# XiSHEN0220/RANSAC-Flow

Measured on NVIDIA H100. Metric: image-pairs/sec at 480x640, nbIter=1k RANSAC, higher is better.
Workload: dtype f32-grade: fp16 hi/lo split operands and activations (22 significand bits), 3 wgmma MMAs per MAC, fp32 accumulate; fp16-split correlation; fp32/fp64 RANSAC

## Files before the change

### ransac-flow_b200/csrc/gemm_tc.cu

```cuda
#include <cuda.h>
#include <cuda_fp16.h>

#include <climits>
#include <mutex>
#include <unordered_map>

#include "common.cuh"
#include "tc_common.cuh"

namespace rf {

constexpr int K_TF32 = 0, K_F16 = 1, K_SPLIT = 2, K_TF32X3 = 3;
constexpr int MODE_CONV = 0, MODE_CORR = 1;
constexpr int O_F32 = 0, O_F16 = 1, O_SPLIT = 2;
constexpr int WG_THREADS = 288;

struct alignas(64) WgParams {
    CUtensorMap mapA[RF_MAX_IMGS];
    CUtensorMap mapA2[RF_MAX_IMGS];
    CUtensorMap mapY[RF_MAX_IMGS];
    CUtensorMap mapR[RF_MAX_IMGS];
    CUtensorMap mapB;
    CUtensorMap mapBlo;
    int nimg;
    int ntiles;
    int tile_start[RF_MAX_IMGS + 1];
    int tiles_x[RF_MAX_IMGS];
    int tw[RF_MAX_IMGS];
    int Ho[RF_MAX_IMGS], Wo[RF_MAX_IMGS];
    long long out_pix[RF_MAX_IMGS + 1];
    int R, S, pad, stride, Cin, Cout, relu, round_out;
    int dil;
    int kc1, stride2;
    long long plane;
    const float* bias;
    const void* residual;
    void* y;
    unsigned long long* rowbest;
    unsigned long long* colbest;
    int NA, NB;
};
static_assert(sizeof(WgParams) <= 32764, "kernel parameter space (CUDA 12.1+ large kernel parameters)");

template <int KIND, int BN, int MODE>
struct WgCfg {
    static constexpr int NPL = (KIND == K_SPLIT || KIND == K_TF32X3) ? 2 : 1;
    static constexpr int A_BYTES = NPL * TC_A_BYTES;
    static constexpr int B_PLANE = BN * 128;
    static constexpr int STAGE_BYTES = A_BYTES + NPL * B_PLANE;
    static constexpr bool ONE_CTA = MODE == MODE_CORR || NPL * BN >= 256;
    static constexpr int BUDGET = ONE_CTA ? 200 * 1024 : 100 * 1024;
    static constexpr int STAGES = BUDGET / STAGE_BYTES > 6 ? 6 : BUDGET / STAGE_BYTES;
    static constexpr int CTAS_PER_SM = ONE_CTA ? 1 : 2;
    static constexpr int SMEM_BYTES = STAGES * STAGE_BYTES + 1024  + 256 ;
    static_assert(STAGES >= 2 && SMEM_BYTES <= 227 * 1024, "shared memory");
};

__device__ __forceinline__ __half2 pack_sat(float a, float b) {
    uint32_t r;
    asm("cvt.rn.satfinite.f16x2.f32 %0, %1, %2;" : "=r"(r) : "f"(b), "f"(a));
    return *reinterpret_cast<__half2*>(&r);
}
__device__ __forceinline__ void split2(float a, float b, __half2& hi, __half2& lo) {
    hi = pack_sat(a, b);
    const float2 f = __half22float2(hi);
    lo = pack_sat((a - f.x) * 2048.f, (b - f.y) * 2048.f);
}

template <int KIND, int BN, int NACC>
__device__ __forceinline__ void mma_block(float (&acc)[NACC][BN / 2], uint32_t sa, uint32_t sb) {
    constexpr bool TF32 = KIND == K_TF32 || KIND == K_TF32X3;
#pragma unroll
    for (int k = 0; k < 4; ++k) {
        const uint64_t ah = wg_desc(sa + 32 * k), bh = wg_desc(sb + 32 * k);
        if constexpr (KIND == K_SPLIT || KIND == K_TF32X3) {
            const uint64_t al = wg_desc(sa + TC_A_BYTES + 32 * k), bl = wg_desc(sb + BN * 128 + 32 * k);
            float (&x)[BN / 2] = acc[NACC - 1];
            wgmma<TF32, BN>(x, al, bh);
            wgmma<TF32, BN>(x, ah, bl);
            wgmma<TF32, BN>(acc[0], ah, bh);
        } else {
            wgmma<TF32, BN>(acc[0], ah, bh);
        }
    }
}

template <int KIND, int BN, int MODE, int OUT>
__global__ void __launch_bounds__(WG_THREADS, WgCfg<KIND, BN, MODE>::CTAS_PER_SM)
wg_kernel(const __grid_constant__ WgParams p) {
    using Cfg = WgCfg<KIND, BN, MODE>;
    constexpr int STAGES = Cfg::STAGES;
    constexpr int BK = (KIND == K_TF32 || KIND == K_TF32X3) ? TC_BK : TC_BK_F16;
    constexpr int NACC = KIND == K_SPLIT ? 2 : 1;
    constexpr bool SLOT = MODE == MODE_CONV && OUT != O_F32;
    constexpr int BOX_BYTES = (OUT == O_SPLIT ? 2 : 1) * 128 * 128;
    static_assert(!SLOT || (BN / 64) * BOX_BYTES <= Cfg::STAGE_BYTES, "the output tile fits one stage");
    extern __shared__ uint8_t smem_raw[];
    uint8_t* smem = smem_raw + ((1024u - (smem_u32(smem_raw) & 1023u)) & 1023u);
    uint64_t* full = reinterpret_cast<uint64_t*>(smem + STAGES * Cfg::STAGE_BYTES);
    uint64_t* empty = full + STAGES;
    const int warp = threadIdx.x >> 5, lane = threadIdx.x & 31;
    const int kc = p.Cin / BK;
    const int KI = p.R * p.S * kc;

    const int t_first = MODE == MODE_CORR ? 0 : (int)blockIdx.x;
    const int t_step = MODE == MODE_CORR ? 1 : (int)gridDim.x;
    const int t_end = MODE == MODE_CORR ? 1 : p.ntiles;
    const int nt = (p.Cout + BN - 1) / BN;
    struct Tile { int img, tw, ox0, oy0, n0; };
    auto decode = [&](int t) {
        const int mtile = MODE == MODE_CORR ? (int)blockIdx.y : t / nt;
        const int ntile = MODE == MODE_CORR ? (int)blockIdx.x : t - mtile * nt;
        Tile T;
        T.img = 0;
#pragma unroll
        for (int j = 1; j < RF_MAX_IMGS; ++j) T.img += (j < p.nimg && mtile >= p.tile_start[j]) ? 1 : 0;
        const int tloc = mtile - p.tile_start[T.img];
        T.tw = p.tw[T.img];
        const int tyi = tloc / p.tiles_x[T.img], txi = tloc - tyi * p.tiles_x[T.img];
        T.ox0 = txi * T.tw;
        T.oy0 = tyi * (128 / T.tw);
        T.n0 = ntile * BN;
        return T;
    };
    auto boxes = [&](const Tile& T) { return BN == 64 || T.n0 + 64 >= p.Cout ? 1 : 2; };

    if (threadIdx.x == 0) {
        for (int s = 0; s < STAGES; ++s) { mbar_init(&full[s], 1); mbar_init(&empty[s], 256); }
        fence_barrier_init();
    }
    __syncthreads();

    if (warp == 8) {
        if (lane == 0) {
            tma_prefetch_desc(&p.mapB);
            uint32_t prefetched = 0;
            int st = 0;
            uint32_t ph = 0;
            for (int t = t_first; t < t_end; t += t_step) {
                const Tile T = decode(t);
                if (!((prefetched >> T.img) & 1u)) {
                    prefetched |= 1u << T.img;
                    tma_prefetch_desc(&p.mapA[T.img]);
                    if constexpr (SLOT) {
                        tma_prefetch_desc(&p.mapY[T.img]);
                        if (p.residual) tma_prefetch_desc(&p.mapR[T.img]);
                    }
                }
                for (int it = 0; it < KI; ++it) {
                    mbar_wait(&empty[st], ph ^ 1);
                    uint8_t* sa = smem + st * Cfg::STAGE_BYTES;
                    uint8_t* sb = sa + Cfg::A_BYTES;
                    mbar_expect_tx(&full[st], Cfg::STAGE_BYTES);
                    if constexpr (MODE == MODE_CORR) {
                        const int c0 = it * BK;
                        tma_load_3d(sa, &p.mapA[0], &full[st], c0, T.ox0, 0);
                        tma_load_3d(sa + TC_A_BYTES, &p.mapA2[0], &full[st], c0, T.ox0, 0);
                        tma_load_2d(sb, &p.mapB, &full[st], c0, T.n0);
                        tma_load_2d(sb + Cfg::B_PLANE, &p.mapBlo, &full[st], c0, T.n0);
                    } else {
                        const int tap = it / kc, cc = it - tap * kc;
                        const int r = tap / p.S, s = tap - r * p.S;
                        const int c0 = cc * BK, x = T.ox0 * p.stride + s * p.dil - p.pad, y = T.oy0 * p.stride + r * p.dil - p.pad;
                        const int kcol = tap * p.Cin + c0;
                        if constexpr (KIND == K_SPLIT) {
                            if (cc < p.kc1) tma_load_4d(sa, &p.mapA[T.img], &full[st], c0, x, y, 0);
                            else tma_load_4d(sa, &p.mapA2[T.img], &full[st], (cc - p.kc1) * BK, T.ox0 * p.stride2, T.oy0 * p.stride2, 0);
                            tma_load_3d(sb, &p.mapB, &full[st], kcol, T.n0, 0);
                        } else {
                            tma_load_3d(sa, &p.mapA[T.img], &full[st], c0, x, y);
                            tma_load_2d(sb, &p.mapB, &full[st], kcol, T.n0);
                        }
                    }
                    if (++st == STAGES) { st = 0; ph ^= 1; }
                }
                if constexpr (SLOT) {
                    mbar_wait(&empty[st], ph ^ 1);
                    if (p.residual) {
                        const int nb = boxes(T);
                        uint8_t* slot = smem + st * Cfg::STAGE_BYTES;
                        mbar_expect_tx(&full[st], nb * BOX_BYTES);
                        for (int b = 0; b < nb; ++b) {
                            if constexpr (OUT == O_SPLIT) tma_load_4d(slot + b * BOX_BYTES, &p.mapR[T.img], &full[st], T.n0 + 64 * b, T.ox0, T.oy0, 0);
                            else tma_load_3d(slot + b * BOX_BYTES, &p.mapR[T.img], &full[st], T.n0 + 64 * b, T.ox0, T.oy0);
                        }
                    } else {
                        mbar_arrive(&full[st]);
                    }
                    if (++st == STAGES) { st = 0; ph ^= 1; }
                }
            }
        }
        return;
    }

    const int g = warp >> 2;
    const int rbase = 64 * g + 16 * (warp & 3) + (lane >> 2);
    const int cbase = 2 * (lane & 3);
    auto before = [](int s) { return s == 0 ? STAGES - 1 : s - 1; };
    int st = 0;
    uint32_t ph = 0;
    bool stored = false;
    for (int t = t_first; t < t_end; t += t_step) {
        const Tile T = decode(t);
        float acc[NACC][BN / 2];
#pragma unroll
        for (int a = 0; a < NACC; ++a)
#pragma unroll
            for (int i = 0; i < BN / 2; ++i) acc[a][i] = 0.f;
        for (int it = 0; it < KI; ++it) {
            mbar_wait(&full[st], ph);
            const uint32_t sa = smem_u32(smem + st * Cfg::STAGE_BYTES);
            wg_fence();
            mma_block<KIND, BN, NACC>(acc, sa + g * (64 * 128), sa + Cfg::A_BYTES);
            wg_commit();
            wg_wait<1>();
            if (it > 0) {
                mbar_arrive(&empty[before(st)]);
            } else if (SLOT && stored) {
                if (threadIdx.x == 0) bulk_wait_read();
                mbar_arrive(&empty[before(st)]);
            }
            if (++st == STAGES) { st = 0; ph ^= 1; }
        }
        wg_wait<0>();
#pragma unroll
        for (int a = 0; a < NACC; ++a) wg_fence_regs(acc[a]);
        mbar_arrive(&empty[before(st)]);

        auto value = [&](int i) -> float {
            if constexpr (KIND == K_SPLIT) return fmaf(acc[1][i], 0.00048828125f, acc[0][i]);
            else return acc[0][i];
        };

        if constexpr (SLOT) {
            mbar_wait(&full[st], ph);
            uint8_t* slot = smem + st * Cfg::STAGE_BYTES;
#pragma unroll
            for (int h = 0; h < 2; ++h) {
                const int m = rbase + 8 * h;
#pragma unroll
                for (int j = 0; j < BN / 8; ++j) {
                    const int c = 8 * j + cbase, n = T.n0 + c;
                    if (n >= p.Cout) continue;
                    float v0 = value(4 * j + 2 * h), v1 = value(4 * j + 2 * h + 1);
                    if (p.bias) { v0 += __ldg(p.bias + n); v1 += __ldg(p.bias + n + 1); }
                    uint8_t* e = slot + (c >> 6) * BOX_BYTES + m * 128 + ((((c & 63) >> 3) ^ (m & 7)) << 4) + (c & 7) * 2;
                    if (p.residual) {
                        if constexpr (OUT == O_F16) {
                            const float2 r = __half22float2(*reinterpret_cast<const __half2*>(e));
                            v0 += r.x; v1 += r.y;
                        } else {
                            const float2 rh = __half22float2(*reinterpret_cast<const __half2*>(e));
                            const float2 rl = __half22float2(*reinterpret_cast<const __half2*>(e + 128 * 128));
                            v0 += fmaf(rl.x, 0.00048828125f, rh.x); v1 += fmaf(rl.y, 0.00048828125f, rh.y);
                        }
                    }
                    if (p.relu) { v0 = fmaxf(v0, 0.f); v1 = fmaxf(v1, 0.f); }
                    if constexpr (OUT == O_F16) {
                        *reinterpret_cast<__half2*>(e) = pack_sat(v0, v1);
                    } else {
                        __half2 hi, lo;
                        split2(v0, v1, hi, lo);
                        *reinterpret_cast<__half2*>(e) = hi;
                        *reinterpret_cast<__half2*>(e + 128 * 128) = lo;
                    }
                }
            }
            fence_proxy_async();
            asm volatile("bar.sync 1, 256;" ::: "memory");
            if (threadIdx.x == 0) {
                const int nb = boxes(T);
                for (int b = 0; b < nb; ++b) {
                    if constexpr (OUT == O_SPLIT) tma_store_4d(&p.mapY[T.img], slot + b * BOX_BYTES, T.n0 + 64 * b, T.ox0, T.oy0, 0);
                    else tma_store_3d(&p.mapY[T.img], slot + b * BOX_BYTES, T.n0 + 64 * b, T.ox0, T.oy0);
                }
                bulk_commit();
            }
            stored = true;
            if (++st == STAGES) { st = 0; ph ^= 1; }
        } else if constexpr (MODE == MODE_CONV) {
            const int img = T.img, tw = T.tw;
#pragma unroll
            for (int h = 0; h < 2; ++h) {
                const int m = rbase + 8 * h;
                const int py = m / tw, px = m - py * tw;
                const int oy = T.oy0 + py, ox = T.ox0 + px;
                if (oy >= p.Ho[img] || ox >= p.Wo[img]) continue;
                const long long pix = p.out_pix[img] + (long long)oy * p.Wo[img] + ox;
#pragma unroll
                for (int j = 0; j < BN / 8; ++j) {
                    const int n = T.n0 + 8 * j + cbase;
                    if (n >= p.Cout) continue;
                    const bool two = n + 1 < p.Cout;
                    float v0 = value(4 * j + 2 * h), v1 = value(4 * j + 2 * h + 1);
                    if (p.bias) { v0 += __ldg(p.bias + n); if (two) v1 += __ldg(p.bias + n + 1); }
                    const long long o = pix * p.Cout + n;
                    if (p.residual) {
                        const float* r = static_cast<const float*>(p.residual) + o;
                        v0 += __ldg(r); if (two) v1 += __ldg(r + 1);
                    }
                    if (p.relu) { v0 = fmaxf(v0, 0.f); v1 = fmaxf(v1, 0.f); }
                    if (p.round_out) { v0 = round_tf32(v0); v1 = round_tf32(v1); }
                    float* y = static_cast<float*>(p.y) + o;
                    if (two && (p.Cout & 1) == 0) *reinterpret_cast<float2*>(y) = make_float2(v0, v1);
                    else { y[0] = v0; if (two) y[1] = v1; }
                }
            }
        } else {
            const int n0 = T.n0;
            unsigned long long* sCol = reinterpret_cast<unsigned long long*>(smem);
            const int row0 = T.ox0 + rbase, row1 = row0 + 8;
            const bool rv0 = row0 < p.NA, rv1 = row1 < p.NA;
            unsigned long long rb0 = 0ull, rb1 = 0ull;
            asm volatile("bar.sync 1, 256;" ::: "memory");
#pragma unroll
            for (int j = 0; j < BN / 8; ++j) {
#pragma unroll
                for (int e = 0; e < 2; ++e) {
                    const int c = 8 * j + cbase + e, col = n0 + c;
                    const bool cv = col < p.NB;
                    const float s0 = value(4 * j + e), s1 = value(4 * j + 2 + e);
                    unsigned long long ck = 0ull;
                    if (cv) {
                        if (rv0) { const unsigned long long k = pack_key(s0, (uint32_t)col); rb0 = k > rb0 ? k : rb0; ck = pack_key(s0, (uint32_t)row0); }
                        if (rv1) { const unsigned long long k = pack_key(s1, (uint32_t)col); rb1 = k > rb1 ? k : rb1;
                                   const unsigned long long k1 = pack_key(s1, (uint32_t)row1); ck = k1 > ck ? k1 : ck; }
                    }
#pragma unroll
                    for (int off = 4; off < 32; off <<= 1) {
                        const unsigned long long o = __shfl_xor_sync(0xffffffffu, ck, off);
                        ck = o > ck ? o : ck;
                    }
                    if (lane < 4) sCol[warp * BN + c] = ck;
                }
            }
#pragma unroll
            for (int off = 1; off < 4; off <<= 1) {
                const unsigned long long o0 = __shfl_xor_sync(0xffffffffu, rb0, off), o1 = __shfl_xor_sync(0xffffffffu, rb1, off);
                rb0 = o0 > rb0 ? o0 : rb0;
                rb1 = o1 > rb1 ? o1 : rb1;
            }
            if ((lane & 3) == 0) {
                if (rv0 && rb0 != 0ull) atomicMax(p.rowbest + row0, rb0);
                if (rv1 && rb1 != 0ull) atomicMax(p.rowbest + row1, rb1);
            }
            asm volatile("bar.sync 1, 256;" ::: "memory");
            for (int c = threadIdx.x; c < BN; c += 256) {
                if (n0 + c >= p.NB) continue;
                unsigned long long cb = 0ull;
#pragma unroll
                for (int w = 0; w < 8; ++w) { const unsigned long long k = sCol[w * BN + c]; cb = k > cb ? k : cb; }
                if (cb != 0ull) atomicMax(p.colbest + n0 + c, cb);
            }
        }
    }
    if constexpr (SLOT)
        if (threadIdx.x == 0) bulk_wait();
}


constexpr int ST_TW = 32, ST_TH = 4, ST_K = 7, ST_C = 3, ST_KK = 147, ST_KB = 3;
constexpr int ST_PW = (ST_TW - 2) / 2, ST_PH = ST_TH / 2;
constexpr int ST_IN_W = ((ST_TW - 1) * 2 + ST_K) * ST_C;
constexpr int ST_IN_H = (ST_TH - 1) * 2 + ST_K;
constexpr int ST_IN_LD = 208;
constexpr int ST_THREADS = 256;
constexpr int ST_B_PLANE = 64 * 128;
constexpr int ST_OFF_ALO = ST_KB * TC_A_BYTES;
constexpr int ST_OFF_B = 2 * ST_KB * TC_A_BYTES;
constexpr int ST_OFF_T = ST_OFF_B + ST_KB * 2 * ST_B_PLANE;
constexpr int ST_T_BYTES = 128 * 64 * 4;
constexpr int ST_OFF_IN = ST_OFF_T + 2 * ST_T_BYTES;
constexpr int ST_OFF_BAR = ST_OFF_IN + ST_IN_H * ST_IN_LD * 4;
constexpr int ST_SMEM = ST_OFF_BAR + 64 + 1024;
constexpr int ST_NLD = (ST_IN_H * ST_IN_W + ST_THREADS - 1) / ST_THREADS;
static_assert(ST_SMEM <= 227 * 1024, "stem shared memory");
static_assert(ST_PH * ST_PW * 8 <= ST_THREADS, "one thread per (pooled pixel, 8 channels) of a step");

struct alignas(64) StemParams {
    CUtensorMap mapB;
    int nimg, pool;
    int unit_start[RF_MAX_IMGS + 1];
    int steps[RF_MAX_IMGS];
    int H[RF_MAX_IMGS], W[RF_MAX_IMGS];
    int Hs[RF_MAX_IMGS], Ws[RF_MAX_IMGS];
    int Ho[RF_MAX_IMGS], Wo[RF_MAX_IMGS];
    long long in_pix[RF_MAX_IMGS], out_pix[RF_MAX_IMGS];
    long long plane;
    const float* x;
    const float* bias;
    __half* y;
};

__device__ __forceinline__ uint32_t stem_pack_split(float v) {
    __half2 hi, lo;
    split2(v, 0.f, hi, lo);
    return (*reinterpret_cast<uint32_t*>(&hi) & 0xFFFFu) | (*reinterpret_cast<uint32_t*>(&lo) << 16);
}

template <bool SPLIT, int HALF, int kb>
__device__ __forceinline__ void stem_build_half(const uint32_t* __restrict__ base, uint8_t* sA, int m) {
#pragma unroll
    for (int cc = 0; cc < 4; ++cc) {
        const int c8 = HALF * 4 + cc;
        uint4 oh, ol;
        uint32_t* ph = reinterpret_cast<uint32_t*>(&oh);
        uint32_t* pl = reinterpret_cast<uint32_t*>(&ol);
#pragma unroll
        for (int e = 0; e < 4; ++e) {
            const int k0 = kb * 64 + c8 * 8 + 2 * e, k1 = k0 + 1;
            const uint32_t a = k0 < ST_KK ? base[(k0 / 21) * ST_IN_LD + (k0 % 21)] : 0u;
            const uint32_t b = k1 < ST_KK ? base[(k1 / 21) * ST_IN_LD + (k1 % 21)] : 0u;
            ph[e] = __byte_perm(a, b, 0x5410);
            pl[e] = __byte_perm(a, b, 0x7632);
        }
        uint8_t* dst = sA + kb * TC_A_BYTES + m * 128 + ((c8 ^ (m & 7)) << 4);
        *reinterpret_cast<uint4*>(dst) = oh;
        if constexpr (SPLIT) *reinterpret_cast<uint4*>(dst + ST_OFF_ALO) = ol;
    }
}

template <bool SPLIT, int kb, int NACC>
__device__ __forceinline__ void stem_kblock(float (&acc)[NACC][32], const uint32_t* base, uint8_t* sA, const uint8_t* sB, int m, int half,
                                            int g, uint64_t* bar_b, bool first) {
    constexpr int NPL = SPLIT ? 2 : 1;
    if (half == 0) stem_build_half<SPLIT, 0, kb>(base, sA, m);
    else stem_build_half<SPLIT, 1, kb>(base, sA, m);
    fence_proxy_async();
    __syncthreads();
    if (kb == 0 && first) mbar_wait(bar_b, 0);
    wg_fence();
    const uint32_t a = smem_u32(sA + kb * TC_A_BYTES + g * (64 * 128)), b = smem_u32(sB + kb * NPL * ST_B_PLANE);
#pragma unroll
    for (int k = 0; k < 4; ++k) {
        const uint64_t ah = wg_desc(a + 32 * k), bh = wg_desc(b + 32 * k);
        if constexpr (SPLIT) {
            wgmma<false, 64>(acc[1], wg_desc(a + ST_OFF_ALO + 32 * k), bh);
            wgmma<false, 64>(acc[1], ah, wg_desc(b + ST_B_PLANE + 32 * k));
        }
        wgmma<false, 64>(acc[0], ah, bh);
    }
    wg_commit();
}

template <bool SPLIT>
__global__ void __launch_bounds__(ST_THREADS, 1)
stem7_kernel(const __grid_constant__ StemParams p) {
    constexpr int NPL = SPLIT ? 2 : 1;
    constexpr int NACC = SPLIT ? 2 : 1;
    constexpr int PIX_BYTES = SPLIT ? 256 : 128;
    extern __shared__ uint8_t smem_raw[];
    uint8_t* smem = smem_raw + ((1024u - (smem_u32(smem_raw) & 1023u)) & 1023u);
    uint8_t* sA = smem;
    uint8_t* sB = smem + ST_OFF_B;
    uint8_t* sT = smem + ST_OFF_T;
    uint32_t* sIn = reinterpret_cast<uint32_t*>(smem + ST_OFF_IN);
    uint64_t* bar_b = reinterpret_cast<uint64_t*>(smem + ST_OFF_BAR);
    const int t = threadIdx.x, warp = t >> 5, lane = t & 31, g = warp >> 2;
    const long long units = p.unit_start[RF_MAX_IMGS];
    const int u_begin = (int)(units * blockIdx.x / gridDim.x), u_end = (int)(units * (blockIdx.x + 1) / gridDim.x);

    struct Unit { int img, strip, j, r0, c0; };
    auto decode = [&](int u) {
        Unit U;
        U.img = 0;
#pragma unroll
        for (int i = 1; i < RF_MAX_IMGS; ++i) U.img += (i < p.nimg && u >= p.unit_start[i]) ? 1 : 0;
        const int loc = u - p.unit_start[U.img];
        U.strip = loc / p.steps[U.img];
        U.j = loc - U.strip * p.steps[U.img];
        U.r0 = U.j * ST_TH;
        U.c0 = p.pool ? U.strip * 2 * ST_PW - 1 : U.strip * ST_TW;
        return U;
    };
    float win[ST_NLD];
    auto load_window = [&](const Unit& U) {
        const int H = p.H[U.img], WC = p.W[U.img] * ST_C;
        const float* src = p.x + p.in_pix[U.img] * ST_C;
        const int iy0 = U.r0 * 2 - 3, col0 = (U.c0 * 2 - 3) * ST_C;
#pragma unroll
        for (int i = 0; i < ST_NLD; ++i) {
            const int idx = t + i * ST_THREADS;
            const int r = idx / ST_IN_W, jj = idx - r * ST_IN_W;
            const int iy = iy0 + r, col = col0 + jj;
            win[i] = (idx < ST_IN_H * ST_IN_W && iy >= 0 && iy < H && col >= 0 && col < WC) ? __ldg(src + (long long)iy * WC + col) : 0.f;
        }
    };
    auto stage_window = [&]() {
#pragma unroll
        for (int i = 0; i < ST_NLD; ++i) {
            const int idx = t + i * ST_THREADS;
            const int r = idx / ST_IN_W, jj = idx - r * ST_IN_W;
            if (idx < ST_IN_H * ST_IN_W) sIn[r * ST_IN_LD + jj] = stem_pack_split(win[i]);
        }
    };

    if (t == 0) {
        mbar_init(bar_b, 1);
        fence_barrier_init();
    }
    __syncthreads();
    if (t == 0) {
        mbar_expect_tx(bar_b, ST_KB * NPL * ST_B_PLANE);
#pragma unroll
        for (int kb = 0; kb < ST_KB; ++kb) {
            if constexpr (SPLIT) tma_load_3d(sB + kb * 2 * ST_B_PLANE, &p.mapB, bar_b, kb * 64, 0, 0);
            else tma_load_2d(sB + kb * ST_B_PLANE, &p.mapB, bar_b, kb * 64, 0);
        }
    }
    int u = u_begin;
    Unit U = decode(u);
    if (p.pool && U.j > 0) U = decode(--u);
    load_window(U);
    stage_window();
    __syncthreads();

    const int m = t & 127, half = t >> 7;
    const uint32_t* base = sIn + (2 * (m >> 5)) * ST_IN_LD + 6 * (m & 31);
    const int rbase = 64 * g + 16 * (warp & 3) + (lane >> 2), cbase = 2 * (lane & 3);
    int buf = 0;
    for (bool first = true; u < u_end; ++u, first = false) {
        float acc[NACC][32];
#pragma unroll
        for (int a = 0; a < NACC; ++a)
#pragma unroll
            for (int i = 0; i < 32; ++i) acc[a][i] = 0.f;
        stem_kblock<SPLIT, 0>(acc, base, sA, sB, m, half, g, bar_b, first);
        stem_kblock<SPLIT, 1>(acc, base, sA, sB, m, half, g, bar_b, first);
        stem_kblock<SPLIT, 2>(acc, base, sA, sB, m, half, g, bar_b, first);
        const bool more = u + 1 < u_end;
        Unit N = U;
        if (more) {
            N = decode(u + 1);
            load_window(N);
        }
        wg_wait<0>();
#pragma unroll
        for (int a = 0; a < NACC; ++a) wg_fence_regs(acc[a]);

        const int img = U.img;
        uint8_t* tile = sT + buf * ST_T_BYTES;
#pragma unroll
        for (int h = 0; h < 2; ++h) {
            const int mm = rbase + 8 * h;
            const int oy = U.r0 + (mm >> 5), ox = U.c0 + (mm & 31);
            __half* y = p.y + (p.out_pix[img] + (long long)oy * p.Wo[img] + ox) * 64;
            const bool store = !p.pool && oy < p.Hs[img] && ox < p.Ws[img];
#pragma unroll
            for (int j = 0; j < 8; ++j) {
                const int n = 8 * j + cbase, i = 4 * j + 2 * h;
                float v0 = SPLIT ? fmaf(acc[NACC - 1][i], 0.00048828125f, acc[0][i]) : acc[0][i];
                float v1 = SPLIT ? fmaf(acc[NACC - 1][i + 1], 0.00048828125f, acc[0][i + 1]) : acc[0][i + 1];
                if (p.bias) { v0 += __ldg(p.bias + n); v1 += __ldg(p.bias + n + 1); }
                v0 = fmaxf(v0, 0.f);
                v1 = fmaxf(v1, 0.f);
                if constexpr (SPLIT) {
                    __half2 hi, lo;
                    split2(v0, v1, hi, lo);
                    if (p.pool) {
                        const float2 fh = __half22float2(hi), fl = __half22float2(lo);
                        *reinterpret_cast<float2*>(tile + mm * PIX_BYTES + (((n >> 2) ^ (mm & 7)) << 4) + (n & 3) * 4) =
                            make_float2(fmaf(fl.x, 0.00048828125f, fh.x), fmaf(fl.y, 0.00048828125f, fh.y));
                    } else if (store) {
                        *reinterpret_cast<__half2*>(y + n) = hi;
                        *reinterpret_cast<__half2*>(y + p.plane + n) = lo;
                    }
                } else {
                    if (p.pool) *reinterpret_cast<__half2*>(tile + mm * PIX_BYTES + ((j ^ (mm & 7)) << 4) + cbase * 2) = pack_sat(v0, v1);
                    else if (store) *reinterpret_cast<__half2*>(y + n) = pack_sat(v0, v1);
                }
            }
        }
        if (more) stage_window();
        __syncthreads();

        if (p.pool && u >= u_begin && t < ST_PH * ST_PW * 8) {
            const int oct = t & 7, q = t >> 3, pr = q / ST_PW, pc = q - pr * ST_PW;
            const int oy = U.j * ST_PH + pr, ox = U.strip * ST_PW + pc;
            if (oy < p.Ho[img] && ox < p.Wo[img]) {
                float mx[8];
#pragma unroll
                for (int e = 0; e < 8; ++e) mx[e] = -INFINITY;
                const __half2 ninf = __float2half2_rn(-INFINITY);
                __half2 mh[4] = {ninf, ninf, ninf, ninf};
#pragma unroll
                for (int r = 0; r < 3; ++r) {
                    const int tr = 2 * pr - 1 + r;
                    if (U.r0 + tr < 0 || U.r0 + tr >= p.Hs[img]) continue;
                    const uint8_t* trow = tr < 0 ? sT + (buf ^ 1) * ST_T_BYTES + 3 * 32 * PIX_BYTES : tile + tr * 32 * PIX_BYTES;
#pragma unroll
                    for (int s = 0; s < 3; ++s) {
                        const int tc = 2 * pc + s;
                        if (U.c0 + tc < 0 || U.c0 + tc >= p.Ws[img]) continue;
                        const uint8_t* px = trow + tc * PIX_BYTES;
                        if constexpr (SPLIT) {
                            const float4 a = *reinterpret_cast<const float4*>(px + (((2 * oct) ^ (tc & 7)) << 4));
                            const float4 b = *reinterpret_cast<const float4*>(px + (((2 * oct + 1) ^ (tc & 7)) << 4));
                            mx[0] = fmaxf(mx[0], a.x); mx[1] = fmaxf(mx[1], a.y); mx[2] = fmaxf(mx[2], a.z); mx[3] = fmaxf(mx[3], a.w);
                            mx[4] = fmaxf(mx[4], b.x); mx[5] = fmaxf(mx[5], b.y); mx[6] = fmaxf(mx[6], b.z); mx[7] = fmaxf(mx[7], b.w);
                        } else {
                            const uint4 v = *reinterpret_cast<const uint4*>(px + ((oct ^ (tc & 7)) << 4));
                            const __half2* hv = reinterpret_cast<const __half2*>(&v);
#pragma unroll
                            for (int e = 0; e < 4; ++e) mh[e] = __hmax2(mh[e], hv[e]);
                        }
                    }
                }
                __half* y = p.y + (p.out_pix[img] + (long long)oy * p.Wo[img] + ox) * 64 + oct * 8;
                if constexpr (SPLIT) {
                    split_store8(y, p.plane, mx);
                } else {
                    uint4 o;
                    __half2* ho = reinterpret_cast<__half2*>(&o);
#pragma unroll
                    for (int e = 0; e < 4; ++e) ho[e] = mh[e];
                    *reinterpret_cast<uint4*>(y) = o;
                }
            }
        }
        buf ^= 1;
        U = N;
    }
}

__global__ void split_tf32_kernel(const float4* __restrict__ x, float4* __restrict__ hi, float4* __restrict__ lo, long long n4) {
    long long i = (long long)blockIdx.x * blockDim.x + threadIdx.x;
    if (i >= n4) return;
    float4 v = __ldg(x + i), h, l;
    h.x = __uint_as_float(__float_as_uint(v.x) & 0xFFFFE000u); l.x = v.x - h.x;
    h.y = __uint_as_float(__float_as_uint(v.y) & 0xFFFFE000u); l.y = v.y - h.y;
    h.z = __uint_as_float(__float_as_uint(v.z) & 0xFFFFE000u); l.z = v.z - h.z;
    h.w = __uint_as_float(__float_as_uint(v.w) & 0xFFFFE000u); l.w = v.w - h.w;
    hi[i] = h;
    lo[i] = l;
}

__global__ void split_f16_all_kernel(const float4* __restrict__ A, const float4* __restrict__ B, uint2* __restrict__ Ahi, uint2* __restrict__ Alo,
                                     uint2* __restrict__ Bhi, uint2* __restrict__ Blo, long long na4, long long nb4,
                                     unsigned long long* __restrict__ keys, long long nkeys) {
    const long long i = (long long)blockIdx.x * blockDim.x + threadIdx.x;
    if (i < nkeys) keys[i] = 0ull;
    if (i >= na4 + nb4) return;
    const bool isA = i < na4;
    const long long k = isA ? i : i - na4;
    const float4 v = __ldg((isA ? A : B) + k);
    const __half2 h0 = __floats2half2_rn(v.x, v.y), h1 = __floats2half2_rn(v.z, v.w);
    const float2 f0 = __half22float2(h0), f1 = __half22float2(h1);
    const __half2 l0 = __floats2half2_rn((v.x - f0.x) * 2048.f, (v.y - f0.y) * 2048.f);
    const __half2 l1 = __floats2half2_rn((v.z - f1.x) * 2048.f, (v.w - f1.y) * 2048.f);
    uint2 ho, lo2;
    ho.x = *reinterpret_cast<const uint32_t*>(&h0); ho.y = *reinterpret_cast<const uint32_t*>(&h1);
    lo2.x = *reinterpret_cast<const uint32_t*>(&l0); lo2.y = *reinterpret_cast<const uint32_t*>(&l1);
    (isA ? Ahi : Bhi)[k] = ho;
    (isA ? Alo : Blo)[k] = lo2;
}

typedef CUresult (*EncodeTiledFn)(CUtensorMap*, CUtensorMapDataType, cuuint32_t, void*, const cuuint64_t*, const cuuint64_t*,
                                  const cuuint32_t*, const cuuint32_t*, CUtensorMapInterleave, CUtensorMapSwizzle,
                                  CUtensorMapL2promotion, CUtensorMapFloatOOBfill);

static EncodeTiledFn get_encode() {
    static EncodeTiledFn fn = nullptr;
    if (!fn) {
        void* ptr = nullptr;
        cudaDriverEntryPointQueryResult q;
        if (cudaGetDriverEntryPoint("cuTensorMapEncodeTiled", &ptr, cudaEnableDefault, &q) == cudaSuccess && q == cudaDriverEntryPointSuccess)
            fn = reinterpret_cast<EncodeTiledFn>(ptr);
    }
    return fn;
}

struct MapKey {
    const void* ptr;
    unsigned long long d0, d1, d2, d3, plane;
    unsigned b0, b1, b2, b3, es, esize;
    bool operator==(const MapKey& o) const {
        return ptr == o.ptr && d0 == o.d0 && d1 == o.d1 && d2 == o.d2 && d3 == o.d3 && plane == o.plane && b0 == o.b0 && b1 == o.b1 && b2 == o.b2 &&
               b3 == o.b3 && es == o.es && esize == o.esize;
    }
};
struct MapKeyHash {
    size_t operator()(const MapKey& k) const {
        size_t h = std::hash<const void*>()(k.ptr);
        auto mix = [&](unsigned long long v) { h ^= std::hash<unsigned long long>()(v) + 0x9e3779b97f4a7c15ull + (h << 6) + (h >> 2); };
        mix(k.d0); mix(k.d1); mix(k.d2); mix(k.d3); mix(k.plane); mix(k.b0); mix(k.b1); mix(k.b2); mix(k.b3); mix(k.es); mix(k.esize);
        return h;
    }
};
static std::mutex g_map_mu;
static std::unordered_map<MapKey, CUtensorMap, MapKeyHash> g_maps;

int get_map4(CUtensorMap* out, const void* ptr, unsigned long long d0, unsigned long long d1, unsigned long long d2, unsigned long long d3,
             unsigned long long plane_bytes, unsigned b0, unsigned b1, unsigned b2, unsigned b3, unsigned es_, unsigned esize) {
    MapKey key{ptr, d0, d1, d2, d3, plane_bytes, b0, b1, b2, b3, es_, esize};
    std::lock_guard<std::mutex> g(g_map_mu);
    auto it = g_maps.find(key);
    if (it != g_maps.end()) { *out = it->second; return 0; }
    EncodeTiledFn enc = get_encode();
    if (!enc) return fail_msg("cuTensorMapEncodeTiled is not available from this driver");
    cuuint64_t dims[4] = {d0, d1, d2, d3};
    cuuint64_t strides[3] = {d0 * (unsigned long long)esize, d0 * d1 * (unsigned long long)esize, plane_bytes};
    cuuint32_t box[4] = {b0, b1 * es_, b2 * es_, b3};
    cuuint32_t es[4] = {1, es_, es_, 1};
    int rank = d3 > 0 ? 4 : (d2 > 0 ? 3 : 2);
    CUresult r = enc(out, esize == 2 ? CU_TENSOR_MAP_DATA_TYPE_FLOAT16 : CU_TENSOR_MAP_DATA_TYPE_FLOAT32, rank, const_cast<void*>(ptr), dims, strides, box, es,
                     CU_TENSOR_MAP_INTERLEAVE_NONE, CU_TENSOR_MAP_SWIZZLE_128B, CU_TENSOR_MAP_L2_PROMOTION_L2_256B,
                     CU_TENSOR_MAP_FLOAT_OOB_FILL_NONE);
    if (r != CUDA_SUCCESS) {
        snprintf(g_err, sizeof(g_err), "cuTensorMapEncodeTiled failed with CUresult %d (dims %llu,%llu,%llu,%llu box %u,%u,%u,%u)", (int)r, d0, d1, d2, d3, b0, b1, b2, b3);
        return 3;
    }
    if (g_maps.size() > 8192) g_maps.clear();
    g_maps[key] = *out;
    return 0;
}

int get_map(CUtensorMap* out, const void* ptr, unsigned long long d0, unsigned long long d1, unsigned long long d2,
            unsigned b0, unsigned b1, unsigned b2, unsigned es_, unsigned esize) {
    return get_map4(out, ptr, d0, d1, d2, 0, 0, b0, b1, b2, 0, es_, esize);
}

int pick_tw(int Ho, int Wo) {
    int best = 16;
    long long best_area = -1;
    const int cands[5] = {16, 32, 8, 64, 128};
    for (int i = 0; i < 5; ++i) {
        int tw = cands[i], th = 128 / tw;
        long long area = (long long)((Wo + tw - 1) / tw) * ((Ho + th - 1) / th);
        if (best_area < 0 || area < best_area) { best_area = area; best = tw; }
    }
    return best;
}

template <int KIND, int BN, int MODE, int OUT>
static int launch_wg(const WgParams& p, dim3 grid, cudaStream_t st) {
    using Cfg = WgCfg<KIND, BN, MODE>;
    static bool attr[64] = {false};
    const int dev = current_device();
    if (!attr[dev]) {
        RF_CUDA(cudaFuncSetAttribute(wg_kernel<KIND, BN, MODE, OUT>, cudaFuncAttributeMaxDynamicSharedMemorySize, Cfg::SMEM_BYTES));
        attr[dev] = true;
    }
    wg_kernel<KIND, BN, MODE, OUT><<<grid, WG_THREADS, Cfg::SMEM_BYTES, st>>>(p);
    RF_LAUNCHED();
    return 0;
}

template <int KIND, int BN, int OUT>
static int launch_conv_bn(const WgParams& p, cudaStream_t st) {
    const int resident = WgCfg<KIND, BN, MODE_CONV>::CTAS_PER_SM * num_sms();
    return launch_wg<KIND, BN, MODE_CONV, OUT>(p, dim3(p.ntiles < resident ? p.ntiles : resident), st);
}
template <int KIND, int OUT>
static int launch_conv(const WgParams& p, int BN, cudaStream_t st) {
    return BN == 128 ? launch_conv_bn<KIND, 128, OUT>(p, st) : launch_conv_bn<KIND, 64, OUT>(p, st);
}

struct SplitDual { const void* x2; const int* hw2; int Cin2, stride2; };

static int conv_impl(const ImgSet& batch, const ConvParams& cp, const void* w, cudaStream_t st, int kind, bool out32, const SplitDual* dual) {
    const bool flat = cp.R == 1 && cp.S == 1 && cp.stride == 1 && cp.pad == 0 && (dual == nullptr || dual->stride2 == 1);
    int hw_flat[2] = {1, 0};
    ImgSet flat_set;
    if (flat) {
        RF_REQUIRE(batch.out_pix[batch.n] <= INT_MAX, "rf_conv2d_nhwc: more than 2^31 - 1 pixels in one batch");
        hw_flat[1] = (int)batch.out_pix[batch.n];
        RF_REQUIRE(make_imgset(flat_set, 1, hw_flat, 1, 1, 0) == 0, "rf_conv2d_nhwc: bad image set");
    }
    const ImgSet& set = flat ? flat_set : batch;
    const int* hw2 = dual == nullptr ? nullptr : flat ? hw_flat : dual->hw2;
    WgParams p;
    memset(&p, 0, sizeof(p));
    const bool split = kind == K_SPLIT;
    const unsigned esz = kind == K_TF32 ? 4u : 2u;
    const unsigned bk = kind == K_TF32 ? TC_BK : TC_BK_F16;
    const int BN = cp.Cout > 64 ? 128 : 64;
    const char* xb = reinterpret_cast<const char*>(cp.x);
    const unsigned long long in_plane = (unsigned long long)set.in_pix[set.n] * cp.Cin * 2ull;
    long long in2_pix[RF_MAX_IMGS + 1] = {0};
    if (dual)
        for (int i = 0; i < set.n; ++i) in2_pix[i + 1] = in2_pix[i] + (long long)hw2[2 * i] * hw2[2 * i + 1];
    const unsigned long long in2_plane = dual ? (unsigned long long)in2_pix[set.n] * dual->Cin2 * 2ull : 0ull;
    p.nimg = set.n;
    const bool tma_out = kind != K_TF32 && !out32;
    const unsigned long long out_plane = (unsigned long long)set.out_pix[set.n] * cp.Cout * 2ull;
    const char* yb = reinterpret_cast<const char*>(cp.y);
    const char* rb = reinterpret_cast<const char*>(cp.residual);
    int tiles = 0;
    for (int i = 0; i < set.n; ++i) {
        const int tw = flat ? 128 : pick_tw(set.Ho[i], set.Wo[i]), th = 128 / tw;
        p.tw[i] = tw;
        p.tiles_x[i] = (set.Wo[i] + tw - 1) / tw;
        p.tile_start[i] = tiles;
        tiles += p.tiles_x[i] * ((set.Ho[i] + th - 1) / th);
        p.Ho[i] = set.Ho[i]; p.Wo[i] = set.Wo[i];
        p.out_pix[i] = set.out_pix[i];
        int rc = split ? get_map4(&p.mapA[i], xb + set.in_pix[i] * cp.Cin * 2, (unsigned long long)cp.Cin, (unsigned long long)set.W[i],
                                  (unsigned long long)set.H[i], 2, in_plane, bk, (unsigned)tw, (unsigned)th, 2, (unsigned)cp.stride, 2)
                       : get_map(&p.mapA[i], xb + set.in_pix[i] * cp.Cin * esz, (unsigned long long)cp.Cin, (unsigned long long)set.W[i],
                                 (unsigned long long)set.H[i], bk, (unsigned)tw, (unsigned)th, (unsigned)cp.stride, esz);
        if (!rc && dual)
            rc = get_map4(&p.mapA2[i], static_cast<const char*>(dual->x2) + in2_pix[i] * dual->Cin2 * 2, (unsigned long long)dual->Cin2,
                          (unsigned long long)hw2[2 * i + 1], (unsigned long long)hw2[2 * i], 2, in2_plane, bk, (unsigned)tw,
                          (unsigned)th, 2, (unsigned)dual->stride2, 2);
        const long long o = set.out_pix[i] * cp.Cout * 2;
        for (int m = 0; m < (cp.residual ? 2 : 1) && tma_out && !rc; ++m) {
            CUtensorMap* map = m == 0 ? &p.mapY[i] : &p.mapR[i];
            const void* base = (m == 0 ? yb : rb) + o;
            rc = split ? get_map4(map, base, (unsigned long long)cp.Cout, (unsigned long long)set.Wo[i], (unsigned long long)set.Ho[i], 2,
                                  out_plane, 64, (unsigned)tw, (unsigned)th, 2, 1, 2)
                       : get_map(map, base, (unsigned long long)cp.Cout, (unsigned long long)set.Wo[i], (unsigned long long)set.Ho[i],
                                 64, (unsigned)tw, (unsigned)th, 1, 2);
        }
        if (rc) return rc;
    }
    RF_REQUIRE(tiles > 0, "rf_conv2d_nhwc: empty output");
    for (int i = set.n; i <= RF_MAX_IMGS; ++i) p.tile_start[i] = tiles;
    p.out_pix[set.n] = set.out_pix[set.n];
    int rc = split ? get_map(&p.mapB, w, (unsigned long long)cp.K, (unsigned long long)cp.Cout, 2, bk, (unsigned)BN, 2, 1, 2)
                   : get_map(&p.mapB, w, (unsigned long long)cp.K, (unsigned long long)cp.Cout, 0, bk, (unsigned)BN, 0, 1, esz);
    if (rc) return rc;
    p.R = cp.R; p.S = cp.S; p.pad = cp.pad; p.stride = cp.stride; p.Cin = cp.Cin; p.Cout = cp.Cout; p.relu = cp.relu; p.round_out = cp.round_out;
    p.dil = cp.dil;
    p.kc1 = cp.Cin / (int)bk;
    p.stride2 = 1;
    if (dual) { p.Cin = cp.Cin + dual->Cin2; p.stride2 = dual->stride2; }
    p.plane = (long long)set.out_pix[set.n] * cp.Cout;
    p.bias = cp.bias; p.residual = cp.residual; p.y = cp.y;
    p.ntiles = tiles * ((cp.Cout + BN - 1) / BN);
    if (kind == K_TF32) return launch_conv<K_TF32, O_F32>(p, BN, st);
    if (kind == K_F16) return out32 ? launch_conv<K_F16, O_F32>(p, BN, st) : launch_conv<K_F16, O_F16>(p, BN, st);
    return out32 ? launch_conv<K_SPLIT, O_F32>(p, BN, st) : launch_conv<K_SPLIT, O_SPLIT>(p, BN, st);
}

template <bool SPLIT>
static int stem_impl(const float* x, int nimg, const int* hw_host, const void* w, const float* bias, void* y, int pool, void* stream) {
    RF_REQUIRE(x != nullptr && w != nullptr && y != nullptr, "rf_stem7: null pointer");
    RF_REQUIRE(((uintptr_t)y % 16) == 0 && ((uintptr_t)w % 16) == 0, "rf_stem7: pointers must be 16-byte aligned");
    ImgSet set;
    RF_REQUIRE(make_imgset(set, nimg, hw_host, 7, 2, 3) == 0, "rf_stem7: bad image set");
    StemParams p;
    memset(&p, 0, sizeof(p));
    p.nimg = nimg;
    p.pool = pool ? 1 : 0;
    int units = 0;
    long long out = 0;
    for (int i = 0; i < nimg; ++i) {
        const int Hs = set.Ho[i], Ws = set.Wo[i];
        const int Ho = pool ? (Hs - 1) / 2 + 1 : Hs, Wo = pool ? (Ws - 1) / 2 + 1 : Ws;
        const int strips = pool ? (Wo + ST_PW - 1) / ST_PW : (Ws + ST_TW - 1) / ST_TW;
        p.steps[i] = pool ? (Ho + ST_PH - 1) / ST_PH : (Hs + ST_TH - 1) / ST_TH;
        p.unit_start[i] = units;
        units += strips * p.steps[i];
        p.H[i] = set.H[i]; p.W[i] = set.W[i]; p.Hs[i] = Hs; p.Ws[i] = Ws; p.Ho[i] = Ho; p.Wo[i] = Wo;
        p.in_pix[i] = set.in_pix[i];
        p.out_pix[i] = out;
        out += (long long)Ho * Wo;
    }
    for (int i = nimg; i <= RF_MAX_IMGS; ++i) p.unit_start[i] = units;
    int rc = SPLIT ? get_map(&p.mapB, w, 192ull, 64ull, 2, 64, 64, 2, 1, 2) : get_map(&p.mapB, w, 192ull, 64ull, 0, 64, 64, 0, 1, 2);
    if (rc) return rc;
    p.plane = out * 64;
    p.x = x; p.bias = bias; p.y = static_cast<__half*>(y);
    static bool attr[64] = {false};
    const int dev = current_device();
    if (!attr[dev]) {
        RF_CUDA(cudaFuncSetAttribute(stem7_kernel<SPLIT>, cudaFuncAttributeMaxDynamicSharedMemorySize, ST_SMEM));
        attr[dev] = true;
    }
    const int grid = units < num_sms() ? units : num_sms();
    stem7_kernel<SPLIT><<<grid, ST_THREADS, ST_SMEM, as_stream(stream)>>>(p);
    RF_LAUNCHED();
    return 0;
}

}

using namespace rf;

bool rf_conv2d_tc_supported(const ConvParams& p) {
    return (p.stride == 1 || p.stride == 2) && (p.Cin % TC_BK) == 0 && p.Cout >= 1 && p.R == p.S && (p.R == 1 || p.R == 3);
}
bool rf_conv2d_f16_supported(const ConvParams& p) {
    return (p.stride == 1 || p.stride == 2) && (p.Cin % TC_BK_F16) == 0 && p.Cout >= 8 && (p.Cout % 8) == 0 && p.R == p.S && (p.R == 1 || p.R == 3);
}
bool rf_conv2d_split_supported(const ConvParams& p) {
    return (p.stride == 1 || p.stride == 2) && (p.Cin % TC_BK_F16) == 0 && p.Cout >= 1 && p.R == p.S && (p.R == 1 || p.R == 3);
}

int rf_conv2d_tc(const ImgSet& set, const ConvParams& cp, const void* w_tc, cudaStream_t st, bool f16, bool out32) {
    RF_REQUIRE(w_tc != nullptr, "rf_conv2d_nhwc: tensor-core engines need w_tc ([Cout][R*S*Cin])");
    RF_REQUIRE(f16 ? rf_conv2d_f16_supported(cp) : rf_conv2d_tc_supported(cp),
               "rf_conv2d_nhwc: tensor-core engines need stride 1 or 2, 1x1 or 3x3, Cin % 32 == 0 (fp16: Cin % 64 == 0, Cout % 8 == 0)");
    RF_REQUIRE(!out32 || (f16 && cp.R == 3 && cp.stride == 1 && cp.pad == 1 && cp.residual == nullptr),
               "rf_conv2d_nhwc: engine 3 (fp16 operands, fp32 output) covers 3x3 / stride 1 / pad 1 layers without residual");
    RF_REQUIRE(!f16 || (((uintptr_t)cp.x % 16) == 0 && ((uintptr_t)cp.y % 16) == 0 && ((uintptr_t)cp.residual % 16) == 0),
               "rf_conv2d_nhwc: engine 2 needs 16-byte aligned x / y / residual");
    return conv_impl(set, cp, w_tc, st, f16 ? K_F16 : K_TF32, out32, nullptr);
}

int rf_conv2d_split(const ImgSet& set, const ConvParams& cp, const void* w_split, cudaStream_t st, bool out32) {
    RF_REQUIRE(w_split != nullptr, "rf_conv2d_nhwc: engine 4 needs the split weights ([2][Cout][R*S*Cin] fp16)");
    RF_REQUIRE(rf_conv2d_split_supported(cp), "rf_conv2d_nhwc: engine 4 needs stride 1 or 2, 1x1 or 3x3, Cin % 64 == 0");
    RF_REQUIRE(out32 || (cp.Cout % 8) == 0, "rf_conv2d_nhwc: engine 4 needs Cout % 8 == 0 for split outputs");
    RF_REQUIRE(!out32 || cp.residual == nullptr, "rf_conv2d_nhwc: engine 4 fp32 outputs take no residual");
    RF_REQUIRE(cp.dil == 1 || (!out32 && cp.R == 3 && cp.stride == 1), "rf_conv2d_nhwc: dilation needs engine 4, a 3x3 kernel and stride 1");
    RF_REQUIRE(((uintptr_t)cp.x % 16) == 0 && ((uintptr_t)cp.y % 16) == 0 && ((uintptr_t)cp.residual % 16) == 0 && ((uintptr_t)w_split % 16) == 0,
               "rf_conv2d_nhwc: engine 4 needs 16-byte aligned pointers");
    return conv_impl(set, cp, w_split, st, K_SPLIT, out32, nullptr);
}

extern "C" int rf_conv1x1_dual_split(const void* x1, const void* x2, int nimg, const int* hw1_host, const int* hw2_host, int Cin1, int Cin2,
                                     int stride2, const void* w_split, const float* bias, int Cout, int relu, void* y, void* stream) {
    RF_REQUIRE(x1 != nullptr && x2 != nullptr && y != nullptr && hw1_host != nullptr && hw2_host != nullptr && w_split != nullptr,
               "rf_conv1x1_dual_split: null pointer");
    RF_REQUIRE(Cin1 >= 1 && Cin2 >= 1 && Cout >= 1, "rf_conv1x1_dual_split: bad channel counts");
    RF_REQUIRE((Cin1 % TC_BK_F16) == 0 && (Cin2 % TC_BK_F16) == 0 && (Cout % 8) == 0 && (stride2 == 1 || stride2 == 2),
               "rf_conv1x1_dual_split: Cin1 % 64 == 0, Cin2 % 64 == 0, Cout % 8 == 0, stride2 1 or 2");
    RF_REQUIRE(((uintptr_t)x1 % 16) == 0 && ((uintptr_t)x2 % 16) == 0 && ((uintptr_t)y % 16) == 0 && ((uintptr_t)w_split % 16) == 0,
               "rf_conv1x1_dual_split: pointers must be 16-byte aligned");
    ImgSet set;
    RF_REQUIRE(make_imgset(set, nimg, hw1_host, 1, 1, 0) == 0, "rf_conv1x1_dual_split: bad image set");
    for (int i = 0; i < nimg; ++i)
        RF_REQUIRE((hw2_host[2 * i] - 1) / stride2 + 1 == set.Ho[i] && (hw2_host[2 * i + 1] - 1) / stride2 + 1 == set.Wo[i],
                   "rf_conv1x1_dual_split: the second input, sampled with stride2, must have the first input's size");
    ConvParams p;
    p.x = static_cast<const float*>(x1); p.w = nullptr; p.bias = bias; p.residual = nullptr; p.y = static_cast<float*>(y);
    p.Cin = Cin1; p.Cout = Cout; p.R = 1; p.S = 1; p.stride = 1; p.pad = 0; p.relu = relu;
    p.round_out = 0;
    p.dil = 1;
    p.Mtot = set.out_pix[nimg];
    p.K = Cin1 + Cin2;
    SplitDual dual{x2, hw2_host, Cin2, stride2};
    return conv_impl(set, p, w_split, as_stream(stream), K_SPLIT, false, &dual);
}

int rf_stem7(ActFormat f, const float* x, int nimg, const int* hw_host, const void* w, const float* bias, int pool, void* y, void* stream) {
    return f == ACT_SPLIT ? stem_impl<true>(x, nimg, hw_host, w, bias, y, pool, stream) : stem_impl<false>(x, nimg, hw_host, w, bias, y, pool, stream);
}

size_t rf_corr_tc_workspace(int NA, int NB, int C) { return 2ull * ((size_t)NA + NB) * C * sizeof(float) + 1024; }

int rf_corr_argmax_tc(const float* featA, int NA, const float* featB, int NB, int C,
                      unsigned long long* rowbest, unsigned long long* colbest, void* ws, cudaStream_t st, int precision,
                      const void* const* presplit) {
    const bool f16 = precision == 2;
    RF_REQUIRE(presplit == nullptr || f16, "rf_corr_mutual_nn: pre-split operands go with the fp16-split kernel (precision 2)");
    RF_REQUIRE((C % (f16 ? TC_BK_F16 : TC_BK)) == 0, "rf_corr_mutual_nn: precision 1 needs C % 32 == 0, precision 2 C % 64 == 0");
    uintptr_t base = (reinterpret_cast<uintptr_t>(ws) + 255) & ~(uintptr_t)255;
    const size_t esz = f16 ? 2 : 4;
    char* Ahi = reinterpret_cast<char*>(base);
    char* Alo = Ahi + (size_t)NA * C * esz;
    char* Bhi = Alo + (size_t)NA * C * esz;
    char* Blo = Bhi + (size_t)NB * C * esz;
    long long na4 = (long long)NA * C / 4, nb4 = (long long)NB * C / 4;
    if (presplit != nullptr) {
        Ahi = const_cast<char*>(static_cast<const char*>(presplit[0]));
        Alo = const_cast<char*>(static_cast<const char*>(presplit[1]));
        Bhi = const_cast<char*>(static_cast<const char*>(presplit[2]));
        Blo = const_cast<char*>(static_cast<const char*>(presplit[3]));
        for (int i = 0; i < 4; ++i) RF_REQUIRE(presplit[i] != nullptr && ((uintptr_t)presplit[i] % 16) == 0, "rf_corr_mutual_nn_presplit: planes must be 16-byte aligned");
    } else if (f16) {
        RF_REQUIRE(colbest == rowbest + NA, "rf_corr_mutual_nn: arg-max keys must be contiguous");
        const long long nkeys = (long long)NA + NB, n = na4 + nb4 > nkeys ? na4 + nb4 : nkeys;
        split_f16_all_kernel<<<(unsigned)((n + 255) / 256), 256, 0, st>>>((const float4*)featA, (const float4*)featB, (uint2*)Ahi, (uint2*)Alo,
                                                                            (uint2*)Bhi, (uint2*)Blo, na4, nb4, rowbest, nkeys);
        RF_LAUNCHED();
    } else {
        split_tf32_kernel<<<(unsigned)((na4 + 255) / 256), 256, 0, st>>>((const float4*)featA, (float4*)Ahi, (float4*)Alo, na4);
        RF_LAUNCHED();
        split_tf32_kernel<<<(unsigned)((nb4 + 255) / 256), 256, 0, st>>>((const float4*)featB, (float4*)Bhi, (float4*)Blo, nb4);
        RF_LAUNCHED();
    }
    constexpr int BN = 128;
    const unsigned bk = f16 ? TC_BK_F16 : TC_BK, es = (unsigned)esz;
    WgParams p;
    memset(&p, 0, sizeof(p));
    p.nimg = 1;
    p.tw[0] = 128;
    p.tiles_x[0] = (NA + 127) / 128;
    for (int i = 1; i <= RF_MAX_IMGS; ++i) p.tile_start[i] = p.tiles_x[0];
    p.Ho[0] = 1; p.Wo[0] = NA;
    int rc = get_map(&p.mapA[0], Ahi, (unsigned long long)C, (unsigned long long)NA, 1, bk, 128, 1, 1, es);
    if (!rc) rc = get_map(&p.mapA2[0], Alo, (unsigned long long)C, (unsigned long long)NA, 1, bk, 128, 1, 1, es);
    if (!rc) rc = get_map(&p.mapB, Bhi, (unsigned long long)C, (unsigned long long)NB, 0, bk, BN, 0, 1, es);
    if (!rc) rc = get_map(&p.mapBlo, Blo, (unsigned long long)C, (unsigned long long)NB, 0, bk, BN, 0, 1, es);
    if (rc) return rc;
    p.R = 1; p.S = 1; p.pad = 0; p.stride = 1; p.Cin = C; p.Cout = NB;
    p.rowbest = rowbest; p.colbest = colbest; p.NA = NA; p.NB = NB;
    const dim3 grid((NB + BN - 1) / BN, p.tiles_x[0]);
    RF_REQUIRE(grid.y <= 65535u, "rf_corr_mutual_nn: NA > 8388480");
    if (f16) return launch_wg<K_SPLIT, BN, MODE_CORR, 0>(p, grid, st);
    return launch_wg<K_TF32X3, BN, MODE_CORR, 0>(p, grid, st);
}
```

### ransac-flow_b200/csrc/runner.cu

```cuda
#include "common.cuh"

using namespace rf;

int rf_maxpool(ActFormat f, const void* x, int nimg, const int* hw_host, int C, int k, int stride, int pad, void* y, void* stream);
int rf_blur(ActFormat f, const void* x, int nimg, const int* hw_host, int C, int stride, void* y, void* stream);
int rf_poolblur(ActFormat f, const void* x, int nimg, const int* hw_host, int C, void* y, void* stream);
int rf_im2col(ActFormat f, const float* x, int nimg, const int* hw_host, int C, int k, int stride, int pad, int Kpad, void* y, void* stream);
int rf_stem7(ActFormat f, const float* x, int nimg, const int* hw_host, const void* w, const float* bias, int pool, void* y, void* stream);
int rf_stem3(const float* x, int nimg, const int* hw_host, const float* w, const float* bias, void* y, void* stream);
int rf_conv2d_nhwc_dil(const float* x, int nimg, const int* hw_host, int Cin, const float* w, const float* w_tc, const float* bias,
                       const float* residual, int Cout, int R, int S, int stride, int pad, int dil, int relu, int engine, float* y, void* stream);

extern "C" int rf_run_layers(const rf_layer_t* L, int n, void* const* slots, int nimg, const int* hw_host, int engine, void* stream) {
    RF_REQUIRE(L != nullptr && n >= 1 && nimg >= 1 && nimg <= RF_MAX_IMGS, "rf_run_layers: bad arguments");
    const ActFormat f = act_format(engine);
    RF_REQUIRE(f != ACT_NONE, "rf_run_layers: layer programs run on engine 0 (fp32), 1 (TF32), 2 (fp16) or 4 (split)");
    static thread_local int hw[RF_MAX_SLOTS][2 * RF_MAX_IMGS];
    bool known[RF_MAX_SLOTS] = {false};
    RF_REQUIRE(L[0].src >= 0 && L[0].src < RF_MAX_SLOTS, "rf_run_layers: bad input slot");
    for (int i = 0; i < 2 * nimg; ++i) hw[L[0].src][i] = hw_host[i];
    known[L[0].src] = true;
    for (int li = 0; li < n; ++li) {
        const rf_layer_t& l = L[li];
        RF_REQUIRE(l.src >= 0 && l.src < RF_MAX_SLOTS && l.dst >= 0 && l.dst < RF_MAX_SLOTS && l.res < RF_MAX_SLOTS, "rf_run_layers: slot index out of range");
        RF_REQUIRE(known[l.src], "rf_run_layers: layer reads a slot nothing has written");
        RF_REQUIRE(l.dst != l.src && l.dst != l.res, "rf_run_layers: in-place layers are not supported");
        const int* shw = hw[l.src];
        const float* x = static_cast<const float*>(slots[l.src]);
        float* y = static_cast<float*>(slots[l.dst]);
        int rc = 0;
        int k = l.k, stride = l.stride, pad = l.pad;
        const int dil = l.dil > 1 ? l.dil : 1;
        RF_REQUIRE(dil == 1 || (l.op == RF_OP_CONV && f == ACT_SPLIT && !(l.flags & RF_LAYER_OUT_F32) && k == 3 && stride == 1),
                   "rf_run_layers: dilation is for RF_OP_CONV 3x3 / stride 1 layers with split outputs on engine 4");
        switch (l.op) {
        case RF_OP_CONV: {
            const bool out32 = (l.flags & RF_LAYER_OUT_F32) != 0;
            const int conv_engine = f == ACT_SPLIT ? (out32 ? RF_ENGINE_SPLIT_OUT32 : RF_ENGINE_SPLIT)
                                    : f == ACT_F16 ? ((l.flags & RF_LAYER_TF32) ? RF_ENGINE_TF32 : out32 ? RF_ENGINE_F16_OUT32 : RF_ENGINE_F16)
                                                   : engine;
            const float* w_tc = conv_engine >= RF_ENGINE_F16 ? static_cast<const float*>(l.w_f16) : l.w_tc;
            const float* res = l.res >= 0 ? static_cast<const float*>(slots[l.res]) : nullptr;
            rc = rf_conv2d_nhwc_dil(x, nimg, shw, l.Cin, l.w, w_tc, l.bias, res, l.Cout, k, k, stride, pad, dil, l.relu, conv_engine, y, stream);
            break;
        }
        case RF_OP_CONV_DUAL:
            RF_REQUIRE(f == ACT_SPLIT, "rf_run_layers: RF_OP_CONV_DUAL needs engine 4");
            RF_REQUIRE(l.src2 >= 0 && l.src2 < RF_MAX_SLOTS && known[l.src2] && l.dst != l.src2 && l.res < 0 && k == 1 && stride == 1 && pad == 0,
                       "rf_run_layers: RF_OP_CONV_DUAL needs a written second input slot, k = 1, stride 1, pad 0, no residual");
            rc = rf_conv1x1_dual_split(x, slots[l.src2], nimg, shw, hw[l.src2], l.Cin, l.Cin2, l.stride2, l.w_f16, l.bias, l.Cout, l.relu, y, stream);
            break;
        case RF_OP_STEM3:
            RF_REQUIRE(f == ACT_SPLIT, "rf_run_layers: RF_OP_STEM3 needs engine 4");
            RF_REQUIRE(l.src == L[0].src && l.Cin == 3 && l.Cout == 64 && k == 3 && stride == 2 && pad == 1 && l.relu,
                       "rf_run_layers: RF_OP_STEM3 is segNet's 3x3 / stride 2 / pad 1, 3 -> 64 stem conv (+ ReLU) on the fp32 input slot");
            rc = rf_stem3(x, nimg, shw, l.w, l.bias, y, stream);
            break;
        case RF_OP_STEM7: {
            RF_REQUIRE(f == ACT_F16 || f == ACT_SPLIT, "rf_run_layers: RF_OP_STEM7 needs engine 2 or 4");
            RF_REQUIRE(l.src == L[0].src && l.Cin == 3 && l.Cout == 64 && k == 7 && stride == 2 && pad == 3 && l.relu,
                       "rf_run_layers: RF_OP_STEM7 is the ResNet-50 stem on the fp32 input slot");
            const bool pool = (l.flags & RF_LAYER_STEM_POOL) != 0;
            const rf_layer_t* mp = pool && li + 1 < n ? &L[li + 1] : nullptr;
            RF_REQUIRE(!pool || (mp != nullptr && mp->op == RF_OP_MAXPOOL && mp->src == l.dst && mp->Cin == 64 && mp->k == 3 && mp->stride == 2 &&
                                 mp->pad == 1 && mp->dst >= 0 && mp->dst < RF_MAX_SLOTS && mp->dst != l.src),
                       "rf_run_layers: RF_LAYER_STEM_POOL needs the next layer to be a 3x3 / stride 2 / pad 1 max-pool of the stem's output");
            rc = rf_stem7(f, x, nimg, shw, l.w_f16, l.bias, pool, pool ? slots[mp->dst] : y, stream);
            if (rc) return rc;
            if (pool) {
                for (int i = 0; i < nimg; ++i)
                    for (int d = 0; d < 2; ++d) hw[mp->dst][2 * i + d] = ((shw[2 * i + d] - 1) / 2 + 1 - 1) / 2 + 1;
                known[mp->dst] = true;
                ++li;
                continue;
            }
            break;
        }
        case RF_OP_MAXPOOL:
            rc = rf_maxpool(f, x, nimg, shw, l.Cin, k, stride, pad, y, stream);
            break;
        case RF_OP_BLUR:
            k = 3; pad = 1;
            rc = rf_blur(f, x, nimg, shw, l.Cin, stride, y, stream);
            break;
        case RF_OP_POOLBLUR:
            k = 4; stride = 2; pad = 1;
            rc = rf_poolblur(f, x, nimg, shw, l.Cin, y, stream);
            break;
        case RF_OP_IM2COL:
            RF_REQUIRE(l.src == L[0].src, "rf_run_layers: im2col reads the fp32 input slot");
            rc = rf_im2col(f, x, nimg, shw, l.Cin, k, stride, pad, l.Cout, y, stream);
            break;
        default:
            return fail_msg("rf_run_layers: unknown op");
        }
        if (rc) return rc;
        for (int i = 0; i < nimg; ++i) {
            hw[l.dst][2 * i] = (shw[2 * i] + 2 * pad - dil * (k - 1) - 1) / stride + 1;
            hw[l.dst][2 * i + 1] = (shw[2 * i + 1] + 2 * pad - dil * (k - 1) - 1) / stride + 1;
        }
        known[l.dst] = true;
    }
    return 0;
}
```

### ransac-flow_b200/csrc/wgmma.cuh

```cuda
#pragma once
#include <stdint.h>

namespace rf {

__device__ __forceinline__ void wgmma_f16_n64(float (&d)[32], uint64_t a, uint64_t b) {
    asm volatile(
        "{\n\t.reg .pred p;\n\tsetp.ne.b32 p, 1, 0;\n\t"
        "wgmma.mma_async.sync.aligned.m64n64k16.f32.f16.f16 {%0, %1, %2, %3, %4, %5, %6, %7, %8, %9, %10, %11, %12, %13, %14, %15, %16, %17, %18, %19, %20, %21, %22, %23, %24, %25, %26, %27, %28, %29, %30, %31}, %32, %33, p, 1, 1, 0, 0;\n\t}"
        : "+f"(d[0]), "+f"(d[1]), "+f"(d[2]), "+f"(d[3]), "+f"(d[4]), "+f"(d[5]), "+f"(d[6]), "+f"(d[7]), "+f"(d[8]), "+f"(d[9]), "+f"(d[10]), "+f"(d[11]), "+f"(d[12]), "+f"(d[13]), "+f"(d[14]), "+f"(d[15]), "+f"(d[16]), "+f"(d[17]), "+f"(d[18]), "+f"(d[19]), "+f"(d[20]), "+f"(d[21]), "+f"(d[22]), "+f"(d[23]), "+f"(d[24]), "+f"(d[25]), "+f"(d[26]), "+f"(d[27]), "+f"(d[28]), "+f"(d[29]), "+f"(d[30]), "+f"(d[31])
        : "l"(a), "l"(b));
}

__device__ __forceinline__ void wgmma_f16_n128(float (&d)[64], uint64_t a, uint64_t b) {
    asm volatile(
        "{\n\t.reg .pred p;\n\tsetp.ne.b32 p, 1, 0;\n\t"
        "wgmma.mma_async.sync.aligned.m64n128k16.f32.f16.f16 {%0, %1, %2, %3, %4, %5, %6, %7, %8, %9, %10, %11, %12, %13, %14, %15, %16, %17, %18, %19, %20, %21, %22, %23, %24, %25, %26, %27, %28, %29, %30, %31, %32, %33, %34, %35, %36, %37, %38, %39, %40, %41, %42, %43, %44, %45, %46, %47, %48, %49, %50, %51, %52, %53, %54, %55, %56, %57, %58, %59, %60, %61, %62, %63}, %64, %65, p, 1, 1, 0, 0;\n\t}"
        : "+f"(d[0]), "+f"(d[1]), "+f"(d[2]), "+f"(d[3]), "+f"(d[4]), "+f"(d[5]), "+f"(d[6]), "+f"(d[7]), "+f"(d[8]), "+f"(d[9]), "+f"(d[10]), "+f"(d[11]), "+f"(d[12]), "+f"(d[13]), "+f"(d[14]), "+f"(d[15]), "+f"(d[16]), "+f"(d[17]), "+f"(d[18]), "+f"(d[19]), "+f"(d[20]), "+f"(d[21]), "+f"(d[22]), "+f"(d[23]), "+f"(d[24]), "+f"(d[25]), "+f"(d[26]), "+f"(d[27]), "+f"(d[28]), "+f"(d[29]), "+f"(d[30]), "+f"(d[31]), "+f"(d[32]), "+f"(d[33]), "+f"(d[34]), "+f"(d[35]), "+f"(d[36]), "+f"(d[37]), "+f"(d[38]), "+f"(d[39]), "+f"(d[40]), "+f"(d[41]), "+f"(d[42]), "+f"(d[43]), "+f"(d[44]), "+f"(d[45]), "+f"(d[46]), "+f"(d[47]), "+f"(d[48]), "+f"(d[49]), "+f"(d[50]), "+f"(d[51]), "+f"(d[52]), "+f"(d[53]), "+f"(d[54]), "+f"(d[55]), "+f"(d[56]), "+f"(d[57]), "+f"(d[58]), "+f"(d[59]), "+f"(d[60]), "+f"(d[61]), "+f"(d[62]), "+f"(d[63])
        : "l"(a), "l"(b));
}

__device__ __forceinline__ void wgmma_tf32_n64(float (&d)[32], uint64_t a, uint64_t b) {
    asm volatile(
        "{\n\t.reg .pred p;\n\tsetp.ne.b32 p, 1, 0;\n\t"
        "wgmma.mma_async.sync.aligned.m64n64k8.f32.tf32.tf32 {%0, %1, %2, %3, %4, %5, %6, %7, %8, %9, %10, %11, %12, %13, %14, %15, %16, %17, %18, %19, %20, %21, %22, %23, %24, %25, %26, %27, %28, %29, %30, %31}, %32, %33, p, 1, 1;\n\t}"
        : "+f"(d[0]), "+f"(d[1]), "+f"(d[2]), "+f"(d[3]), "+f"(d[4]), "+f"(d[5]), "+f"(d[6]), "+f"(d[7]), "+f"(d[8]), "+f"(d[9]), "+f"(d[10]), "+f"(d[11]), "+f"(d[12]), "+f"(d[13]), "+f"(d[14]), "+f"(d[15]), "+f"(d[16]), "+f"(d[17]), "+f"(d[18]), "+f"(d[19]), "+f"(d[20]), "+f"(d[21]), "+f"(d[22]), "+f"(d[23]), "+f"(d[24]), "+f"(d[25]), "+f"(d[26]), "+f"(d[27]), "+f"(d[28]), "+f"(d[29]), "+f"(d[30]), "+f"(d[31])
        : "l"(a), "l"(b));
}

__device__ __forceinline__ void wgmma_tf32_n128(float (&d)[64], uint64_t a, uint64_t b) {
    asm volatile(
        "{\n\t.reg .pred p;\n\tsetp.ne.b32 p, 1, 0;\n\t"
        "wgmma.mma_async.sync.aligned.m64n128k8.f32.tf32.tf32 {%0, %1, %2, %3, %4, %5, %6, %7, %8, %9, %10, %11, %12, %13, %14, %15, %16, %17, %18, %19, %20, %21, %22, %23, %24, %25, %26, %27, %28, %29, %30, %31, %32, %33, %34, %35, %36, %37, %38, %39, %40, %41, %42, %43, %44, %45, %46, %47, %48, %49, %50, %51, %52, %53, %54, %55, %56, %57, %58, %59, %60, %61, %62, %63}, %64, %65, p, 1, 1;\n\t}"
        : "+f"(d[0]), "+f"(d[1]), "+f"(d[2]), "+f"(d[3]), "+f"(d[4]), "+f"(d[5]), "+f"(d[6]), "+f"(d[7]), "+f"(d[8]), "+f"(d[9]), "+f"(d[10]), "+f"(d[11]), "+f"(d[12]), "+f"(d[13]), "+f"(d[14]), "+f"(d[15]), "+f"(d[16]), "+f"(d[17]), "+f"(d[18]), "+f"(d[19]), "+f"(d[20]), "+f"(d[21]), "+f"(d[22]), "+f"(d[23]), "+f"(d[24]), "+f"(d[25]), "+f"(d[26]), "+f"(d[27]), "+f"(d[28]), "+f"(d[29]), "+f"(d[30]), "+f"(d[31]), "+f"(d[32]), "+f"(d[33]), "+f"(d[34]), "+f"(d[35]), "+f"(d[36]), "+f"(d[37]), "+f"(d[38]), "+f"(d[39]), "+f"(d[40]), "+f"(d[41]), "+f"(d[42]), "+f"(d[43]), "+f"(d[44]), "+f"(d[45]), "+f"(d[46]), "+f"(d[47]), "+f"(d[48]), "+f"(d[49]), "+f"(d[50]), "+f"(d[51]), "+f"(d[52]), "+f"(d[53]), "+f"(d[54]), "+f"(d[55]), "+f"(d[56]), "+f"(d[57]), "+f"(d[58]), "+f"(d[59]), "+f"(d[60]), "+f"(d[61]), "+f"(d[62]), "+f"(d[63])
        : "l"(a), "l"(b));
}

template <bool TF32, int N>
__device__ __forceinline__ void wgmma(float (&d)[N / 2], uint64_t a, uint64_t b) {
    if constexpr (TF32) { if constexpr (N == 64) wgmma_tf32_n64(d, a, b); else wgmma_tf32_n128(d, a, b); }
    else { if constexpr (N == 64) wgmma_f16_n64(d, a, b); else wgmma_f16_n128(d, a, b); }
}

}
```

### ransac-flow_b200/model.py

```python
import torch
import torch.nn as nn

from . import ops
from .ops import Ragged
from .program import LayerProgram

_engine = ops.ENGINE_FP32


def set_engine(engine):
    global _engine, _fine_f16
    _fine_f16 = engine != "f16-trunk"
    _engine = ({"fp32": ops.ENGINE_FP32, "tf32": ops.ENGINE_TF32, "f16": ops.ENGINE_F16, "f16-trunk": ops.ENGINE_F16,
                "f16x3": ops.ENGINE_SPLIT}[engine] if isinstance(engine, str) else int(engine))


def get_engine():
    return _engine


_fine_f16 = True


def fine_engine():
    return _engine if (_engine != ops.ENGINE_F16 or _fine_f16) else ops.ENGINE_TF32


def conv3x3(in_planes, out_planes, stride=1):
    return nn.Conv2d(in_planes, out_planes, kernel_size=3, stride=stride, padding=1, bias=False)


def conv1x1(in_planes, out_planes, stride=1):
    return nn.Conv2d(in_planes, out_planes, kernel_size=1, stride=stride, bias=False)


def _init_like_reference(module):
    for m in module.modules():
        if isinstance(m, nn.Conv2d):
            nn.init.kaiming_normal_(m.weight, mode="fan_out", nonlinearity="relu")
        elif isinstance(m, nn.BatchNorm2d):
            nn.init.constant_(m.weight, 1)
            nn.init.constant_(m.bias, 0)


class FoldedConv:

    def __init__(self, weight, bn=None, stride=1, pad=None, eps=None, cin_pad=None, device=None):
        dev = weight.device if device is None else torch.device(device)
        w = weight.detach().float().cpu()
        if cin_pad is not None and cin_pad > w.shape[1]:
            w = torch.nn.functional.pad(w, (0, 0, 0, 0, 0, cin_pad - w.shape[1]))
        cout, cin, k, _ = w.shape
        if bn is not None:
            e = bn.eps if eps is None else eps
            scale = bn.weight.detach().float().cpu() / torch.sqrt(bn.running_var.detach().float().cpu() + e)
            self.bias = (bn.bias.detach().float().cpu() - bn.running_mean.detach().float().cpu() * scale).contiguous().to(dev)
            w = w * scale.view(-1, 1, 1, 1)
        else:
            self.bias = None
        self.w = w.permute(2, 3, 1, 0).reshape(k * k * cin, cout).contiguous().to(dev)
        wt = w.permute(0, 2, 3, 1).reshape(cout, k * k * cin).contiguous()
        bits = wt.view(torch.int32)
        bits = (bits + 0xFFF + ((bits >> 13) & 1)) & ~0x1FFF
        self.w_tc = bits.view(torch.float32).contiguous().to(dev)
        self._wt = wt
        self._dev = dev
        self._w_f16 = None
        self.cout, self.cin, self.k, self.stride = cout, cin, k, stride
        self.pad = (k // 2) if pad is None else pad

    @classmethod
    def concat_k(cls, fa, fb):
        assert fa.k == 1 and fb.k == 1 and fa.cout == fb.cout and fa.pad == 0 and fb.pad == 0
        f = cls.__new__(cls)
        f._wt = torch.cat([fa._wt, fb._wt], dim=1).contiguous()
        f._dev, f._w_f16 = fa._dev, None
        f.w = torch.cat([fa.w, fb.w], dim=0).contiguous()
        f.w_tc = torch.cat([fa.w_tc, fb.w_tc], dim=1).contiguous()
        ba = fa.bias if fa.bias is not None else torch.zeros(fa.cout, device=fa._dev)
        f.bias = (ba + fb.bias) if fb.bias is not None else ba
        f.cout, f.cin, f.cin2, f.k, f.stride, f.pad = fa.cout, fa.cin, fb.cin, 1, 1, 0
        return f

    @property
    def w_split(self):
        if getattr(self, "_w_split", None) is None:
            hi = self._wt.to(torch.float16)
            lo = ((self._wt - hi.float()) * 2048.0).to(torch.float16)
            self._w_split = torch.stack([hi, lo]).contiguous().to(self._dev)
        return self._w_split

    @property
    def w_f16(self):
        if self._w_f16 is None:
            self._w_f16 = self._wt.to(torch.float16).contiguous().to(self._dev)
        return self._w_f16

    def __call__(self, x, relu, residual=None, engine=None):
        eng = min(fine_engine(), ops.ENGINE_TF32) if engine is None else engine
        if int(eng) == ops.ENGINE_SPLIT:
            return ops.conv2d(x, self.w, self.bias, self.cout, self.k, self.stride, self.pad, relu, residual, eng, self.w_split)
        return ops.conv2d(x, self.w, self.bias, self.cout, self.k, self.stride, self.pad, relu, residual, eng, self.w_tc)


class _Engine(nn.Module):

    def _folded(self, f16=False):
        f16 = 2 if f16 is True else (int(f16) if int(f16) in (ops.ENGINE_F16, ops.ENGINE_SPLIT) else 0)
        ver = tuple((p._version, p.data_ptr()) for p in list(self.parameters()) + list(self.buffers()))
        if getattr(self, "_fold_ver", None) != ver:
            self._fold = {}
            self._fold_ver = ver
        if f16 not in self._fold:
            with torch.no_grad():
                self._fold[f16] = self._fold_build(f16)
        return self._fold[f16]

    def _check(self, *xs):
        if self.training:
            raise RuntimeError("ransac_flow_b200.model is inference-only: call .eval() first (training is out of scope)")
        for x in xs:
            ops.need_cuda(x)


class Downsample(nn.Module):

    def __init__(self, pad_type="reflect", filt_size=3, stride=2, channels=None, pad_off=0):
        super().__init__()
        assert filt_size == 3 and pad_type in ("refl", "reflect") and pad_off == 0, "only the configuration the hot path uses"
        self.stride, self.channels = stride, channels
        a = torch.tensor([1.0, 2.0, 1.0])
        filt = a[:, None] * a[None, :]
        self.register_buffer("filt", (filt / filt.sum())[None, None].repeat(channels, 1, 1, 1))


class BasicBlock(nn.Module):
    expansion = 1

    def __init__(self, inplanes, planes, stride=1, downsample=None):
        super().__init__()
        self.conv1 = conv3x3(inplanes, planes, stride)
        self.bn1 = nn.BatchNorm2d(planes, eps=1e-05)
        self.conv2 = conv3x3(planes, planes)
        self.bn2 = nn.BatchNorm2d(planes, eps=1e-05)
        self.downsample = downsample
        self.stride = stride


class FeatureExtractor(_Engine):

    def __init__(self):
        super().__init__()
        self.inplanes = 64
        self.conv1 = nn.Conv2d(3, 64, kernel_size=3, stride=1, padding=1, bias=False)
        self.bn1 = nn.BatchNorm2d(64, eps=1e-05)
        self.maxpool = nn.Sequential(nn.MaxPool2d(kernel_size=2, stride=1), Downsample(filt_size=3, stride=2, channels=64))
        self.layer1 = self._make_layer(BasicBlock, 64, 2)
        self.layer2 = self._make_layer(BasicBlock, 128, 2, stride=2)
        self.layer3 = self._make_layer(BasicBlock, 256, 2, stride=2)
        _init_like_reference(self)

    def _make_layer(self, block, planes, blocks, stride=1):
        downsample = None
        if stride != 1 or self.inplanes != planes * block.expansion:
            downsample = [Downsample(filt_size=3, stride=stride, channels=self.inplanes)] if stride != 1 else []
            downsample += [conv1x1(self.inplanes, planes * block.expansion, 1), nn.BatchNorm2d(planes * block.expansion)]
            downsample = nn.Sequential(*downsample)
        layers = [block(self.inplanes, planes, stride, downsample)]
        self.inplanes = planes * block.expansion
        for _ in range(1, blocks):
            layers.append(block(self.inplanes, planes, 1, None))
        return nn.Sequential(*layers)

    def _fold_build(self, f16=False):
        P = LayerProgram(3)
        x = P.stem(0, self.conv1.weight, self.bn1, 1, 1, 64 if f16 else 32)
        x = P.poolblur(x)
        for layer in (self.layer1, self.layer2, self.layer3):
            for b in layer:
                out = P.conv(x, FoldedConv(b.conv1.weight, b.bn1, b.stride), relu=True)
                r = x
                if b.downsample is not None:
                    mods = list(b.downsample)
                    if isinstance(mods[0], Downsample):
                        r = P.blur(r, mods[0].stride)
                    r = P.conv(r, FoldedConv(mods[-2].weight, mods[-1], 1, pad=0), relu=False)
                x = P.conv(out, FoldedConv(b.conv2.weight, b.bn2, 1), relu=True, res=r)
        return P

    def forward_ragged(self, x):
        eng = fine_engine()
        out, ohw = self._folded(eng).run(x, eng)
        return Ragged(out, ohw)

    def forward(self, x):
        self._check(x)
        with torch.no_grad():
            r = self.forward_ragged(Ragged.from_nchw(x))
            if r.split:
                r = Ragged(ops.from_split(r.data), r.hw)
            return r.to_nchw().float().clone(memory_format=torch.channels_last)


class CorrNeigh(nn.Module):

    def __init__(self, kernelSize):
        super().__init__()
        assert kernelSize % 2 == 1
        self.kernelSize = kernelSize
        self.paddingSize = kernelSize // 2

    def forward(self, x, y):
        ops.need_cuda(x, y)
        with torch.no_grad():
            return ops.corr_neigh(Ragged.from_nchw(x), Ragged.from_nchw(y), self.kernelSize).to_nchw()


class _Head(_Engine):
    def __init__(self, kernelSize, cout):
        super().__init__()
        assert kernelSize % 2 == 1
        self.conv1 = conv3x3(kernelSize * kernelSize, 512)
        self.bn1 = nn.BatchNorm2d(512, eps=1e-05)
        self.conv2 = conv3x3(512, 256)
        self.bn2 = nn.BatchNorm2d(256, eps=1e-05)
        self.conv3 = conv3x3(256, 128)
        self.bn3 = nn.BatchNorm2d(128, eps=1e-05)
        self.conv4 = conv3x3(128, cout)
        self.kernelSize = kernelSize
        self.paddingSize = kernelSize // 2
        _init_like_reference(self)

    CORR_LD = 64

    def _fold_build(self, f16=False):
        P = LayerProgram(self.CORR_LD)
        split = f16 == 4
        x = P.conv(0, FoldedConv(self.conv1.weight, self.bn1, cin_pad=self.CORR_LD), relu=True)
        x = P.conv(x, FoldedConv(self.conv2.weight, self.bn2), relu=True)
        x = P.conv(x, FoldedConv(self.conv3.weight, self.bn3), relu=True, out_f32=not split)
        P.conv(x, FoldedConv(self.conv4.weight, None), relu=False, tf32=not split, out_f32=split)
        return P

    def _padded(self, corr, dtype, split=False):
        if corr.C == self.CORR_LD and corr.data.dtype == dtype and corr.split == split:
            return corr
        if split:
            src = ops.from_split(corr.data) if corr.split else corr.data.float()
            d = torch.zeros((src.shape[0], self.CORR_LD), device=src.device, dtype=torch.float32)
            d[:, :min(src.shape[1], self.kernelSize ** 2)] = src[:, :self.kernelSize ** 2]
            return Ragged(ops.to_split(d), corr.hw)
        d = torch.zeros((corr.data.shape[0], self.CORR_LD), device=corr.data.device, dtype=dtype)
        d[:, :min(corr.C, self.kernelSize ** 2)] = corr.data[:, :self.kernelSize ** 2].to(dtype)
        return Ragged(d, corr.hw)

    def trunk(self, corr):
        eng = fine_engine()
        f16, split = eng == ops.ENGINE_F16, eng == ops.ENGINE_SPLIT
        corr = self._padded(corr, torch.float16 if (f16 or split) else torch.float32, split)
        out, ohw = self._folded(eng).run(corr, eng)
        return Ragged(out, ohw)


class NetFlowCoarse(_Head):

    def __init__(self, kernelSize):
        super().__init__(kernelSize, kernelSize * kernelSize)
        r = self.paddingSize
        self.gridY = torch.arange(-r, r + 1).view(1, 1, -1, 1).expand(1, 1, kernelSize, kernelSize).contiguous().view(1, -1, 1, 1).float()
        self.gridX = torch.arange(-r, r + 1).view(1, 1, 1, -1).expand(1, 1, kernelSize, kernelSize).contiguous().view(1, -1, 1, 1).float()

    def cuda(self, device=None):
        super().cuda(device)
        self.gridX, self.gridY = self.gridX.cuda(), self.gridY.cuda()
        return self

    def forward_ragged(self, corr):
        return ops.softmax_flow(self.trunk(corr), self.kernelSize)

    def forward(self, coef, up8X=True):
        self._check(coef)
        with torch.no_grad():
            flow = self.forward_ragged(Ragged.from_nchw(coef))
            if up8X:
                flow = torch.nn.functional.interpolate(flow, scale_factor=8, mode="bilinear", align_corners=True)
            return flow


class NetMatchability(_Head):

    def __init__(self, kernelSize):
        super().__init__(kernelSize, 1)
        nn.init.normal_(self.conv4.weight, mean=0.0, std=0.0001)

    def forward_ragged(self, corr):
        x = self.trunk(corr)
        h, w = corr.hw[0]
        return ops.sigmoid(x.data).view(corr.n, 1, h, w)

    def forward(self, feat, up8X=True):
        self._check(feat)
        with torch.no_grad():
            m = self.forward_ragged(Ragged.from_nchw(feat))
            if up8X:
                m = torch.nn.functional.interpolate(m, scale_factor=8, mode="bilinear", align_corners=True)
            return m


def predFlowCoarse(corrKernel21, NetFlowCoarse, grid, up8X=True):
    flowCoarse = NetFlowCoarse(corrKernel21, up8X)
    b, _, w, h = flowCoarse.size()
    flowGrad = flowCoarse.narrow(2, 1, w - 1).narrow(3, 1, h - 1) - flowCoarse.narrow(2, 0, w - 1).narrow(3, 0, h - 1)
    flowGrad = torch.norm(flowGrad, dim=1, keepdim=True)
    flowCoarse = flowCoarse.permute(0, 2, 3, 1)
    flowCoarse = torch.clamp(flowCoarse + grid, min=-1, max=1)
    return flowGrad, flowCoarse


def predFlowCoarseNoGrad(corrKernel21, NetFlowCoarse, grid, up8X=True):
    flowCoarse = NetFlowCoarse(corrKernel21, up8X).permute(0, 2, 3, 1)
    return torch.clamp(flowCoarse + grid, min=-1, max=1)


def predMatchability(corrKernel21, NetMatchability, up8X=True):
    return NetMatchability(corrKernel21, up8X)
```

### ransac-flow_b200/program.py

```python
import ctypes as C

import torch

from ._lib import check, lib, need_cuda, stream

RF_OP_CONV, RF_OP_MAXPOOL, RF_OP_BLUR, RF_OP_IM2COL, RF_OP_POOLBLUR, RF_OP_STEM7, RF_OP_CONV_DUAL, RF_OP_STEM3 = 0, 1, 2, 3, 4, 5, 6, 7
RF_MAX_SLOTS = 32
RF_LAYER_OUT_F32, RF_LAYER_TF32, RF_LAYER_STEM_POOL = 1, 2, 4


class rf_layer_t(C.Structure):
    _fields_ = [("op", C.c_int), ("src", C.c_int), ("dst", C.c_int), ("res", C.c_int),
                ("Cin", C.c_int), ("Cout", C.c_int), ("k", C.c_int), ("stride", C.c_int), ("pad", C.c_int), ("relu", C.c_int),
                ("w", C.c_void_p), ("w_tc", C.c_void_p), ("bias", C.c_void_p), ("w_f16", C.c_void_p), ("flags", C.c_int),
                ("src2", C.c_int), ("Cin2", C.c_int), ("stride2", C.c_int), ("dil", C.c_int)]


lib.rf_run_layers.restype = C.c_int
lib.rf_run_layers.argtypes = [C.POINTER(rf_layer_t), C.c_int, C.POINTER(C.c_void_p), C.c_int, C.POINTER(C.c_int), C.c_int, C.c_void_p]


class LayerProgram:

    def __init__(self, cin, device=None):
        self.device = device
        self.ops = []
        self.chan = [cin]
        self._keep = []
        self.flags = {}
        self.dual = {}
        self.dil = {}
        self._compiled = {}

    def conv(self, src, fc, relu, res=None, out_f32=False, tf32=False, dil=1):
        assert self.chan[src] == fc.cin, (self.chan[src], fc.cin)
        if dil > 1:
            assert fc.k == 3 and fc.stride == 1 and not (out_f32 or tf32), "dilation: 3x3 / stride 1 layers with split outputs"
            self.split_only = True
        self.dil[len(self.ops)] = int(dil)
        self.flags[len(self.ops)] = (RF_LAYER_OUT_F32 if out_f32 else 0) | (RF_LAYER_TF32 if tf32 else 0)
        self.ops.append((RF_OP_CONV, src, -1 if res is None else res, fc.cin, fc.cout, fc.k, fc.stride, fc.pad, int(relu), fc))
        self._keep.append(fc)
        self.chan.append(fc.cout)
        return len(self.chan) - 1

    def conv_dual(self, src, src2, fc, stride2, relu):
        assert fc.k == 1 and self.chan[src] == fc.cin and self.chan[src2] == fc.cin2, (self.chan[src], self.chan[src2], fc.cin, fc.cin2)
        self.dual[len(self.ops)] = (src2, fc.cin2, stride2)
        self.ops.append((RF_OP_CONV_DUAL, src, -1, fc.cin, fc.cout, 1, 1, 0, int(relu), fc))
        self._keep.append(fc)
        self.chan.append(fc.cout)
        self.split_only = True
        return len(self.chan) - 1

    def maxpool(self, src, k, stride, pad):
        c = self.chan[src]
        self.ops.append((RF_OP_MAXPOOL, src, -1, c, c, k, stride, pad, 0, None))
        self.chan.append(c)
        return len(self.chan) - 1

    def poolblur(self, src):
        c = self.chan[src]
        self.ops.append((RF_OP_POOLBLUR, src, -1, c, c, 4, 2, 1, 0, None))
        self.chan.append(c)
        return len(self.chan) - 1

    def im2col(self, src, k, stride, pad, kpad):
        c = self.chan[src]
        assert kpad >= k * k * c
        self.ops.append((RF_OP_IM2COL, src, -1, c, kpad, k, stride, pad, 0, None))
        self.chan.append(kpad)
        return len(self.chan) - 1

    def stem(self, src, weight, bn, stride, pad, kalign=32):
        from .model import FoldedConv
        cout, cin, k, _ = weight.shape
        kpad = (k * k * cin + kalign - 1) // kalign * kalign
        dev = self.device or weight.device
        w = weight.detach().float().cpu().permute(0, 2, 3, 1).reshape(cout, k * k * cin)
        w = torch.nn.functional.pad(w, (0, kpad - k * k * cin)).reshape(cout, kpad, 1, 1)
        x = self.im2col(src, k, stride, pad, kpad)
        return self.conv(x, FoldedConv(w, bn, 1, pad=0, device=dev), relu=True)

    def stem7_fused(self, src, weight, bn):
        from .model import FoldedConv
        cout, cin, k, _ = weight.shape
        assert (cout, cin, k) == (64, 3, 7) and self.chan[src] == 3
        dev = self.device or weight.device
        w = weight.detach().float().cpu().permute(0, 2, 3, 1).reshape(cout, k * k * cin)
        w = torch.nn.functional.pad(w, (0, 192 - k * k * cin)).reshape(cout, 192, 1, 1)
        fc = FoldedConv(w, bn, 1, pad=0, device=dev)
        self.ops.append((RF_OP_STEM7, src, -1, 3, 64, 7, 2, 3, 1, fc))
        self._keep.append(fc)
        self.chan.append(64)
        self.f16_only = True
        return len(self.chan) - 1

    def stem3(self, src, weight, bn):
        from .model import FoldedConv
        assert tuple(weight.shape) == (64, 3, 3, 3) and self.chan[src] == 3
        fc = FoldedConv(weight, bn, 2, pad=1, device=self.device or weight.device)
        self.ops.append((RF_OP_STEM3, src, -1, 3, 64, 3, 2, 1, 1, fc))
        self._keep.append(fc)
        self.chan.append(64)
        self.split_only = True
        return len(self.chan) - 1

    def blur(self, src, stride):
        c = self.chan[src]
        self.ops.append((RF_OP_BLUR, src, -1, c, c, 3, stride, 1, 0, None))
        self.chan.append(c)
        return len(self.chan) - 1

    def _compile(self, hw, device, f16=False, split=False):
        n_t = len(self.chan)
        last_use = [0] * n_t
        for i, o in enumerate(self.ops):
            last_use[o[1]] = i
            if o[2] >= 0:
                last_use[o[2]] = i
            if i in self.dual:
                last_use[self.dual[i][0]] = i
        last_use[n_t - 1] = len(self.ops)
        hws = [list(hw)]
        for i, o in enumerate(self.ops):
            k, s, p, d = o[5], o[6], o[7], self.dil.get(i, 1)
            hws.append([((h + 2 * p - d * (k - 1) - 1) // s + 1, (w + 2 * p - d * (k - 1) - 1) // s + 1) for h, w in hws[o[1]]])
        esize = [4] * n_t
        if f16:
            esize[0] = 4 if self.ops[0][0] in (RF_OP_IM2COL, RF_OP_STEM7) else 2
            for i, o in enumerate(self.ops):
                fl = self.flags.get(i, 0)
                esize[i + 1] = 4 if fl else 2
                if fl & RF_LAYER_TF32:
                    assert esize[o[1]] == 4, "a TF32 layer under the fp16 engine needs an fp32 input (out_f32 on its producer)"
                elif o[0] not in (RF_OP_IM2COL, RF_OP_STEM7):
                    assert esize[o[1]] == 2 and (o[2] < 0 or esize[o[2]] == 2), "fp16 layer fed by an fp32 tensor"
        elems = [sum(h * w for h, w in hws[t]) * self.chan[t] * esize[t] for t in range(n_t)]
        stem_pool = set()
        for i, o in enumerate(self.ops[:-1]):
            q = self.ops[i + 1]
            if (f16 or split) and o[0] == RF_OP_STEM7 and q[0] == RF_OP_MAXPOOL and q[1] == i + 1 and tuple(q[5:8]) == (3, 2, 1) \
                    and last_use[i + 1] == i + 1:
                stem_pool.add(i)
                elems[i + 1] = 0
        slot_of, free, slot_elems = {0: 0}, [], [0]
        layers = (rf_layer_t * len(self.ops))()
        for i, o in enumerate(self.ops):
            t_out = i + 1
            if free:
                fit = [s for s in free if slot_elems[s] >= elems[t_out]]
                s = min(fit, key=lambda q: slot_elems[q]) if fit else max(free, key=lambda q: slot_elems[q])
                free.remove(s)
                slot_elems[s] = max(slot_elems[s], elems[t_out])
            else:
                s = len(slot_elems)
                slot_elems.append(elems[t_out])
            slot_of[t_out] = s
            L = layers[i]
            L.op, L.src, L.dst, L.res = o[0], slot_of[o[1]], s, (slot_of[o[2]] if o[2] >= 0 else -1)
            L.Cin, L.Cout, L.k, L.stride, L.pad, L.relu = o[3], o[4], o[5], o[6], o[7], o[8]
            fc = o[9]
            if fc is not None:
                L.w, L.w_tc = fc.w.data_ptr(), fc.w_tc.data_ptr()
                L.w_f16 = fc.w_f16.data_ptr() if f16 else (fc.w_split.data_ptr() if split else None)
                L.flags = (self.flags.get(i, 0) | (RF_LAYER_STEM_POOL if i in stem_pool else 0)) if (f16 or split) else 0
                L.bias = fc.bias.data_ptr() if fc.bias is not None else None
            L.src2 = -1
            L.dil = self.dil.get(i, 1)
            if i in self.dual:
                L.src2, L.Cin2, L.stride2 = slot_of[self.dual[i][0]], self.dual[i][1], self.dual[i][2]
            for t in {o[1], o[2], self.dual[i][0] if i in self.dual else -1}:
                if t > 0 and last_use[t] == i:
                    free.append(slot_of[t])
        assert len(slot_elems) <= RF_MAX_SLOTS
        bufs = [None] + [torch.empty(max(16, e), device=device, dtype=torch.uint8) for e in slot_elems[1:]]
        out_slot = slot_of[n_t - 1]
        chw = (C.c_int * (2 * len(hw)))(*[v for p in hw for v in p])
        out_split = split and not (self.flags.get(len(self.ops) - 1, 0) & RF_LAYER_OUT_F32)
        in_split = split and self.ops[0][0] not in (RF_OP_IM2COL, RF_OP_STEM7, RF_OP_STEM3)
        return dict(layers=layers, bufs=bufs, out_slot=out_slot, out_hw=hws[-1], out_elems=elems[-1], chw=chw, nslots=len(slot_elems),
                    out_dtype=torch.float16 if (esize[-1] == 2 or out_split) else torch.float32, out_split=out_split,
                    in_dtype=torch.float16 if (esize[0] == 2 or in_split) else torch.float32)

    def run(self, x, engine):
        need_cuda(x.data)
        f16, split = int(engine) == 2, int(engine) == 4
        assert f16 or split or not getattr(self, "f16_only", False), "this program uses tensor-core-engine-only layers"
        assert split or not getattr(self, "split_only", False), "this program uses split-engine-only layers (conv_dual, dilation)"
        key = (tuple(x.hw), str(x.data.device), int(engine) if (f16 or split) else 0)
        if key not in self._compiled:
            self._compiled[key] = self._compile(x.hw, x.data.device, f16, split)
        c = self._compiled[key]
        self.__dict__.setdefault("_touched", set()).add(key)
        assert x.data.dtype == c["in_dtype"], (x.data.dtype, c["in_dtype"])
        slots = (C.c_void_p * c["nslots"])()
        slots[0] = x.data.data_ptr()
        for i in range(1, c["nslots"]):
            slots[i] = c["bufs"][i].data_ptr()
        check(lib.rf_run_layers(c["layers"], len(self.ops), slots, len(x.hw), c["chw"], int(engine), stream()))
        out = c["bufs"][c["out_slot"]][:c["out_elems"]].view(c["out_dtype"])
        out = out.view(2, -1, self.chan[-1]) if c["out_split"] else out.view(-1, self.chan[-1])
        return out, c["out_hw"]

    def release(self, keep=()):
        for k in [k for k in self._compiled if k not in keep]:
            del self._compiled[k]
```

Measured before the change: 141.6.

## Generalize fused stem kernel to 3x3 stride-1 and route FeatureExtractor stem through it

Templates the fused stem kernel on kernel size and stride so the FeatureExtractor's 3x3/stride-1 conv uses the fused path instead of a separate im2col plus GEMM in the f16 build. The A operand is now gathered straight into registers through a precomputed offset table and fed to register-sourced wgmma, with the gather for the next k-step overlapped with the current MMA. The input window is double-buffered, and unpooled outputs are staged in a swizzled shared tile and written with 16-byte coalesced stores. The stride-1 variant runs two CTAs per SM. The risks are higher register pressure and a bug that only shows in the new stride-1 geometry.

```diff
diff --git a/ransac-flow_b200/csrc/gemm_tc.cu b/ransac-flow_b200/csrc/gemm_tc.cu
--- a/ransac-flow_b200/csrc/gemm_tc.cu
+++ b/ransac-flow_b200/csrc/gemm_tc.cu
@@ -360,23 +360,37 @@
 }
 
 
-constexpr int ST_TW = 32, ST_TH = 4, ST_K = 7, ST_C = 3, ST_KK = 147, ST_KB = 3;
+constexpr int ST_TW = 32, ST_TH = 4, ST_C = 3;
 constexpr int ST_PW = (ST_TW - 2) / 2, ST_PH = ST_TH / 2;
-constexpr int ST_IN_W = ((ST_TW - 1) * 2 + ST_K) * ST_C;
-constexpr int ST_IN_H = (ST_TH - 1) * 2 + ST_K;
-constexpr int ST_IN_LD = 208;
 constexpr int ST_THREADS = 256;
 constexpr int ST_B_PLANE = 64 * 128;
-constexpr int ST_OFF_ALO = ST_KB * TC_A_BYTES;
-constexpr int ST_OFF_B = 2 * ST_KB * TC_A_BYTES;
-constexpr int ST_OFF_T = ST_OFF_B + ST_KB * 2 * ST_B_PLANE;
 constexpr int ST_T_BYTES = 128 * 64 * 4;
-constexpr int ST_OFF_IN = ST_OFF_T + 2 * ST_T_BYTES;
-constexpr int ST_OFF_BAR = ST_OFF_IN + ST_IN_H * ST_IN_LD * 4;
-constexpr int ST_SMEM = ST_OFF_BAR + 64 + 1024;
-constexpr int ST_NLD = (ST_IN_H * ST_IN_W + ST_THREADS - 1) / ST_THREADS;
-static_assert(ST_SMEM <= 227 * 1024, "stem shared memory");
 static_assert(ST_PH * ST_PW * 8 <= ST_THREADS, "one thread per (pooled pixel, 8 channels) of a step");
+
+template <int KS, int S>
+struct StemGeo {
+    static constexpr int PAD = (KS - 1) / 2;
+    static constexpr int KK = KS * KS * ST_C;
+    static constexpr int KSTEPS = (KK + 15) / 16;
+    static constexpr int KB = (KSTEPS + 3) / 4;
+    static constexpr int IN_H = (ST_TH - 1) * S + KS;
+    static constexpr int IN_COLS = (ST_TW - 1) * S + KS;
+    static constexpr int IN_W = IN_COLS * ST_C;
+    static constexpr int EVEN_W = (IN_COLS + 1) / 2 * ST_C;
+    static constexpr int LD = S == 2 ? 208 : 104;
+    static constexpr int WIN = IN_H * LD;
+    static constexpr int NLD = (IN_H * IN_W + ST_THREADS - 1) / ST_THREADS;
+    static constexpr int NT = S == 2 ? 3 : 2;
+    static constexpr int CTAS = S == 2 ? 1 : 2;
+    static constexpr int OFF_T = KB * 2 * ST_B_PLANE;
+    static constexpr int OFF_IN = OFF_T + NT * ST_T_BYTES;
+    static constexpr int OFF_K = OFF_IN + 2 * WIN * 4;
+    static constexpr int OFF_BAR = OFF_K + KSTEPS * 4 * 16;
+    static constexpr int SMEM = OFF_BAR + 64 + 1024;
+    static_assert(LD >= (S == 2 ? EVEN_W + IN_COLS / 2 * ST_C : IN_W), "window row");
+    static_assert(CTAS * SMEM <= 227 * 1024, "stem shared memory");
+    static __device__ __forceinline__ int word(int r, int ix, int c) { return r * LD + (S == 2 ? (ix & 1) * EVEN_W + (ix >> 1) * ST_C : ix * ST_C) + c; }
+};
 
 struct alignas(64) StemParams {
     CUtensorMap mapB;
@@ -399,64 +413,63 @@
     return (*reinterpret_cast<uint32_t*>(&hi) & 0xFFFFu) | (*reinterpret_cast<uint32_t*>(&lo) << 16);
 }
 
-template <bool SPLIT, int HALF, int kb>
-__device__ __forceinline__ void stem_build_half(const uint32_t* __restrict__ base, uint8_t* sA, int m) {
-#pragma unroll
-    for (int cc = 0; cc < 4; ++cc) {
-        const int c8 = HALF * 4 + cc;
-        uint4 oh, ol;
-        uint32_t* ph = reinterpret_cast<uint32_t*>(&oh);
-        uint32_t* pl = reinterpret_cast<uint32_t*>(&ol);
-#pragma unroll
-        for (int e = 0; e < 4; ++e) {
-            const int k0 = kb * 64 + c8 * 8 + 2 * e, k1 = k0 + 1;
-            const uint32_t a = k0 < ST_KK ? base[(k0 / 21) * ST_IN_LD + (k0 % 21)] : 0u;
-            const uint32_t b = k1 < ST_KK ? base[(k1 / 21) * ST_IN_LD + (k1 % 21)] : 0u;
-            ph[e] = __byte_perm(a, b, 0x5410);
-            pl[e] = __byte_perm(a, b, 0x7632);
-        }
-        uint8_t* dst = sA + kb * TC_A_BYTES + m * 128 + ((c8 ^ (m & 7)) << 4);
-        *reinterpret_cast<uint4*>(dst) = oh;
-        if constexpr (SPLIT) *reinterpret_cast<uint4*>(dst + ST_OFF_ALO) = ol;
-    }
-}
-
-template <bool SPLIT, int kb, int NACC>
-__device__ __forceinline__ void stem_kblock(float (&acc)[NACC][32], const uint32_t* base, uint8_t* sA, const uint8_t* sB, int m, int half,
-                                            int g, uint64_t* bar_b, bool first) {
-    constexpr int NPL = SPLIT ? 2 : 1;
-    if (half == 0) stem_build_half<SPLIT, 0, kb>(base, sA, m);
-    else stem_build_half<SPLIT, 1, kb>(base, sA, m);
-    fence_proxy_async();
-    __syncthreads();
-    if (kb == 0 && first) mbar_wait(bar_b, 0);
-    wg_fence();
-    const uint32_t a = smem_u32(sA + kb * TC_A_BYTES + g * (64 * 128)), b = smem_u32(sB + kb * NPL * ST_B_PLANE);
-#pragma unroll
-    for (int k = 0; k < 4; ++k) {
-        const uint64_t ah = wg_desc(a + 32 * k), bh = wg_desc(b + 32 * k);
+struct StemFrag { uint32_t h[4], l[4]; };
+
+template <int KK, int j>
+__device__ __forceinline__ void stem_gather(StemFrag& f, const uint32_t* __restrict__ w, int base, const int4* sK, int q) {
+    const int4 o4 = sK[j * 4 + q];
+    const int o[4] = {o4.x, o4.y, o4.z, o4.w};
+    uint32_t v[2][4];
+#pragma unroll
+    for (int h = 0; h < 2; ++h)
+#pragma unroll
+        for (int e = 0; e < 4; ++e) v[h][e] = (16 * (j + 1) <= KK || o[e] >= 0) ? w[base + 24 * h + o[e]] : 0u;
+#pragma unroll
+    for (int e = 0; e < 2; ++e)
+#pragma unroll
+        for (int h = 0; h < 2; ++h) {
+            f.h[2 * e + h] = __byte_perm(v[h][2 * e], v[h][2 * e + 1], 0x5410);
+            f.l[2 * e + h] = __byte_perm(v[h][2 * e], v[h][2 * e + 1], 0x7632);
+        }
+}
+
+template <int KK, int KSTEPS, bool SPLIT, int j, int NACC>
+__device__ __forceinline__ void stem_mma(float (&acc)[NACC][32], StemFrag (&buf)[2], const uint32_t* w, int base, const int4* sK, int q,
+                                         uint32_t sB) {
+    if constexpr (j < KSTEPS) {
+        constexpr int NPL = SPLIT ? 2 : 1;
+        StemFrag& f = buf[j & 1];
+        wg_fence();
+        const uint32_t b = sB + (j >> 2) * NPL * ST_B_PLANE + 32 * (j & 3);
+        const uint64_t bh = wg_desc(b);
         if constexpr (SPLIT) {
-            wgmma<false, 64>(acc[1], wg_desc(a + ST_OFF_ALO + 32 * k), bh);
-            wgmma<false, 64>(acc[1], ah, wg_desc(b + ST_B_PLANE + 32 * k));
-        }
-        wgmma<false, 64>(acc[0], ah, bh);
-    }
-    wg_commit();
-}
-
-template <bool SPLIT>
-__global__ void __launch_bounds__(ST_THREADS, 1)
-stem7_kernel(const __grid_constant__ StemParams p) {
+            wgmma_f16_n64_rs(acc[1], f.l, bh);
+            wgmma_f16_n64_rs(acc[1], f.h, wg_desc(b + ST_B_PLANE));
+        }
+        wgmma_f16_n64_rs(acc[0], f.h, bh);
+        wg_commit();
+        if constexpr (j + 1 < KSTEPS) {
+            wg_wait<1>();
+            stem_gather<KK, j + 1>(buf[(j + 1) & 1], w, base, sK, q);
+        }
+        stem_mma<KK, KSTEPS, SPLIT, j + 1>(acc, buf, w, base, sK, q, sB);
+    }
+}
+
+template <int KS, int S, bool SPLIT>
+__global__ void __launch_bounds__(ST_THREADS, StemGeo<KS, S>::CTAS)
+stem_kernel(const __grid_constant__ StemParams p) {
+    using G = StemGeo<KS, S>;
     constexpr int NPL = SPLIT ? 2 : 1;
     constexpr int NACC = SPLIT ? 2 : 1;
     constexpr int PIX_BYTES = SPLIT ? 256 : 128;
     extern __shared__ uint8_t smem_raw[];
     uint8_t* smem = smem_raw + ((1024u - (smem_u32(smem_raw) & 1023u)) & 1023u);
-    uint8_t* sA = smem;
-    uint8_t* sB = smem + ST_OFF_B;
-    uint8_t* sT = smem + ST_OFF_T;
-    uint32_t* sIn = reinterpret_cast<uint32_t*>(smem + ST_OFF_IN);
-    uint64_t* bar_b = reinterpret_cast<uint64_t*>(smem + ST_OFF_BAR);
+    uint8_t* sB = smem;
+    uint8_t* sT = smem + G::OFF_T;
+    uint32_t* sIn = reinterpret_cast<uint32_t*>(smem + G::OFF_IN);
+    int4* sK = reinterpret_cast<int4*>(smem + G::OFF_K);
+    uint64_t* bar_b = reinterpret_cast<uint64_t*>(smem + G::OFF_BAR);
     const int t = threadIdx.x, warp = t >> 5, lane = t & 31, g = warp >> 2;
     const long long units = p.unit_start[RF_MAX_IMGS];
     const int u_begin = (int)(units * blockIdx.x / gridDim.x), u_end = (int)(units * (blockIdx.x + 1) / gridDim.x);
@@ -474,25 +487,25 @@
         U.c0 = p.pool ? U.strip * 2 * ST_PW - 1 : U.strip * ST_TW;
         return U;
     };
-    float win[ST_NLD];
+    float win[G::NLD];
     auto load_window = [&](const Unit& U) {
         const int H = p.H[U.img], WC = p.W[U.img] * ST_C;
         const float* src = p.x + p.in_pix[U.img] * ST_C;
-        const int iy0 = U.r0 * 2 - 3, col0 = (U.c0 * 2 - 3) * ST_C;
-#pragma unroll
-        for (int i = 0; i < ST_NLD; ++i) {
+        const int iy0 = U.r0 * S - G::PAD, col0 = (U.c0 * S - G::PAD) * ST_C;
+#pragma unroll
+        for (int i = 0; i < G::NLD; ++i) {
             const int idx = t + i * ST_THREADS;
-            const int r = idx / ST_IN_W, jj = idx - r * ST_IN_W;
+            const int r = idx / G::IN_W, jj = idx - r * G::IN_W;
             const int iy = iy0 + r, col = col0 + jj;
-            win[i] = (idx < ST_IN_H * ST_IN_W && iy >= 0 && iy < H && col >= 0 && col < WC) ? __ldg(src + (long long)iy * WC + col) : 0.f;
+            win[i] = (idx < G::IN_H * G::IN_W && iy >= 0 && iy < H && col >= 0 && col < WC) ? __ldg(src + (long long)iy * WC + col) : 0.f;
         }
     };
-    auto stage_window = [&]() {
-#pragma unroll
-        for (int i = 0; i < ST_NLD; ++i) {
+    auto stage_window = [&](uint32_t* dst) {
+#pragma unroll
+        for (int i = 0; i < G::NLD; ++i) {
             const int idx = t + i * ST_THREADS;
-            const int r = idx / ST_IN_W, jj = idx - r * ST_IN_W;
-            if (idx < ST_IN_H * ST_IN_W) sIn[r * ST_IN_LD + jj] = stem_pack_split(win[i]);
+            const int r = idx / G::IN_W, jj = idx - r * G::IN_W, ix = jj / ST_C;
+            if (idx < G::IN_H * G::IN_W) dst[G::word(r, ix, jj - ix * ST_C)] = stem_pack_split(win[i]);
         }
     };
 
@@ -500,11 +513,22 @@
         mbar_init(bar_b, 1);
         fence_barrier_init();
     }
+    if (t < G::KSTEPS * 4) {
+        const int j = t >> 2, q = t & 3;
+        int o[4];
+#pragma unroll
+        for (int e = 0; e < 4; ++e) {
+            const int k = 16 * j + 2 * q + (e & 1) + 8 * (e >> 1);
+            const int r = k / (KS * ST_C), rs = k - r * KS * ST_C, s = rs / ST_C;
+            o[e] = k < G::KK ? G::word(r, s, rs - s * ST_C) : -1;
+        }
+        sK[t] = make_int4(o[0], o[1], o[2], o[3]);
+    }
     __syncthreads();
     if (t == 0) {
-        mbar_expect_tx(bar_b, ST_KB * NPL * ST_B_PLANE);
-#pragma unroll
-        for (int kb = 0; kb < ST_KB; ++kb) {
+        mbar_expect_tx(bar_b, G::KB * NPL * ST_B_PLANE);
+#pragma unroll
+        for (int kb = 0; kb < G::KB; ++kb) {
             if constexpr (SPLIT) tma_load_3d(sB + kb * 2 * ST_B_PLANE, &p.mapB, bar_b, kb * 64, 0, 0);
             else tma_load_2d(sB + kb * ST_B_PLANE, &p.mapB, bar_b, kb * 64, 0);
         }
@@ -513,22 +537,25 @@
     Unit U = decode(u);
     if (p.pool && U.j > 0) U = decode(--u);
     load_window(U);
-    stage_window();
+    stage_window(sIn);
     __syncthreads();
 
-    const int m = t & 127, half = t >> 7;
-    const uint32_t* base = sIn + (2 * (m >> 5)) * ST_IN_LD + 6 * (m & 31);
-    const int rbase = 64 * g + 16 * (warp & 3) + (lane >> 2), cbase = 2 * (lane & 3);
-    int buf = 0;
+    const int q = lane & 3;
+    const int rbase = 64 * g + 16 * (warp & 3) + (lane >> 2), cbase = 2 * q;
+    const int base = (rbase >> 5) * S * G::LD + 3 * (rbase & 31);
+    const uint32_t sB32 = smem_u32(sB);
+    int wb = 0, tb = 0;
     for (bool first = true; u < u_end; ++u, first = false) {
+        const uint32_t* w = sIn + wb * G::WIN;
         float acc[NACC][32];
 #pragma unroll
         for (int a = 0; a < NACC; ++a)
 #pragma unroll
             for (int i = 0; i < 32; ++i) acc[a][i] = 0.f;
-        stem_kblock<SPLIT, 0>(acc, base, sA, sB, m, half, g, bar_b, first);
-        stem_kblock<SPLIT, 1>(acc, base, sA, sB, m, half, g, bar_b, first);
-        stem_kblock<SPLIT, 2>(acc, base, sA, sB, m, half, g, bar_b, first);
+        StemFrag frag[2];
+        stem_gather<G::KK, 0>(frag[0], w, base, sK, q);
+        if (first) mbar_wait(bar_b, 0);
+        stem_mma<G::KK, G::KSTEPS, SPLIT, 0>(acc, frag, w, base, sK, q, sB32);
         const bool more = u + 1 < u_end;
         Unit N = U;
         if (more) {
@@ -540,13 +567,10 @@
         for (int a = 0; a < NACC; ++a) wg_fence_regs(acc[a]);
 
         const int img = U.img;
-        uint8_t* tile = sT + buf * ST_T_BYTES;
+        uint8_t* tile = sT + tb * ST_T_BYTES;
 #pragma unroll
         for (int h = 0; h < 2; ++h) {
             const int mm = rbase + 8 * h;
-            const int oy = U.r0 + (mm >> 5), ox = U.c0 + (mm & 31);
-            __half* y = p.y + (p.out_pix[img] + (long long)oy * p.Wo[img] + ox) * 64;
-            const bool store = !p.pool && oy < p.Hs[img] && ox < p.Ws[img];
 #pragma unroll
             for (int j = 0; j < 8; ++j) {
                 const int n = 8 * j + cbase, i = 4 * j + 2 * h;
@@ -555,6 +579,7 @@
                 if (p.bias) { v0 += __ldg(p.bias + n); v1 += __ldg(p.bias + n + 1); }
                 v0 = fmaxf(v0, 0.f);
                 v1 = fmaxf(v1, 0.f);
+                uint8_t* e = tile + mm * 128 + ((j ^ (mm & 7)) << 4) + cbase * 2;
                 if constexpr (SPLIT) {
                     __half2 hi, lo;
                     split2(v0, v1, hi, lo);
@@ -562,22 +587,30 @@
                         const float2 fh = __half22float2(hi), fl = __half22float2(lo);
                         *reinterpret_cast<float2*>(tile + mm * PIX_BYTES + (((n >> 2) ^ (mm & 7)) << 4) + (n & 3) * 4) =
                             make_float2(fmaf(fl.x, 0.00048828125f, fh.x), fmaf(fl.y, 0.00048828125f, fh.y));
-                    } else if (store) {
-                        *reinterpret_cast<__half2*>(y + n) = hi;
-                        *reinterpret_cast<__half2*>(y + p.plane + n) = lo;
+                    } else {
+                        *reinterpret_cast<__half2*>(e) = hi;
+                        *reinterpret_cast<__half2*>(e + 128 * 128) = lo;
                     }
                 } else {
-                    if (p.pool) *reinterpret_cast<__half2*>(tile + mm * PIX_BYTES + ((j ^ (mm & 7)) << 4) + cbase * 2) = pack_sat(v0, v1);
-                    else if (store) *reinterpret_cast<__half2*>(y + n) = pack_sat(v0, v1);
+                    *reinterpret_cast<__half2*>(e) = pack_sat(v0, v1);
                 }
             }
         }
-        if (more) stage_window();
+        if (more) stage_window(sIn + (wb ^ 1) * G::WIN);
         __syncthreads();
 
-        if (p.pool && u >= u_begin && t < ST_PH * ST_PW * 8) {
-            const int oct = t & 7, q = t >> 3, pr = q / ST_PW, pc = q - pr * ST_PW;
+        if (!p.pool) {
+            for (int i = t; i < NPL * 128 * 8; i += ST_THREADS) {
+                const int pl = i >> 10, mm = (i >> 3) & 127, ch = i & 7;
+                const int oy = U.r0 + (mm >> 5), ox = U.c0 + (mm & 31);
+                if (oy < p.Ho[img] && ox < p.Wo[img])
+                    *reinterpret_cast<uint4*>(p.y + pl * p.plane + (p.out_pix[img] + (long long)oy * p.Wo[img] + ox) * 64 + ch * 8) =
+                        *reinterpret_cast<const uint4*>(tile + pl * 128 * 128 + mm * 128 + ((ch ^ (mm & 7)) << 4));
+            }
+        } else if (u >= u_begin && t < ST_PH * ST_PW * 8) {
+            const int oct = t & 7, qq = t >> 3, pr = qq / ST_PW, pc = qq - pr * ST_PW;
             const int oy = U.j * ST_PH + pr, ox = U.strip * ST_PW + pc;
+            const uint8_t* prev = sT + (tb == 0 ? G::NT - 1 : tb - 1) * ST_T_BYTES;
             if (oy < p.Ho[img] && ox < p.Wo[img]) {
                 float mx[8];
 #pragma unroll
@@ -588,7 +621,7 @@
                 for (int r = 0; r < 3; ++r) {
                     const int tr = 2 * pr - 1 + r;
                     if (U.r0 + tr < 0 || U.r0 + tr >= p.Hs[img]) continue;
-                    const uint8_t* trow = tr < 0 ? sT + (buf ^ 1) * ST_T_BYTES + 3 * 32 * PIX_BYTES : tile + tr * 32 * PIX_BYTES;
+                    const uint8_t* trow = tr < 0 ? prev + 3 * 32 * PIX_BYTES : tile + tr * 32 * PIX_BYTES;
 #pragma unroll
                     for (int s = 0; s < 3; ++s) {
                         const int tc = 2 * pc + s;
@@ -619,7 +652,8 @@
                 }
             }
         }
-        buf ^= 1;
+        wb ^= 1;
+        tb = tb + 1 == G::NT ? 0 : tb + 1;
         U = N;
     }
 }
@@ -834,12 +868,13 @@
     return out32 ? launch_conv<K_SPLIT, O_F32>(p, BN, st) : launch_conv<K_SPLIT, O_SPLIT>(p, BN, st);
 }
 
-template <bool SPLIT>
+template <int KS, int S, bool SPLIT>
 static int stem_impl(const float* x, int nimg, const int* hw_host, const void* w, const float* bias, void* y, int pool, void* stream) {
-    RF_REQUIRE(x != nullptr && w != nullptr && y != nullptr, "rf_stem7: null pointer");
-    RF_REQUIRE(((uintptr_t)y % 16) == 0 && ((uintptr_t)w % 16) == 0, "rf_stem7: pointers must be 16-byte aligned");
+    using G = StemGeo<KS, S>;
+    RF_REQUIRE(x != nullptr && w != nullptr && y != nullptr, "rf_stem: null pointer");
+    RF_REQUIRE(((uintptr_t)y % 16) == 0 && ((uintptr_t)w % 16) == 0, "rf_stem: pointers must be 16-byte aligned");
     ImgSet set;
-    RF_REQUIRE(make_imgset(set, nimg, hw_host, 7, 2, 3) == 0, "rf_stem7: bad image set");
+    RF_REQUIRE(make_imgset(set, nimg, hw_host, KS, S, G::PAD) == 0, "rf_stem: bad image set");
     StemParams p;
     memset(&p, 0, sizeof(p));
     p.nimg = nimg;
@@ -859,18 +894,19 @@
         out += (long long)Ho * Wo;
     }
     for (int i = nimg; i <= RF_MAX_IMGS; ++i) p.unit_start[i] = units;
-    int rc = SPLIT ? get_map(&p.mapB, w, 192ull, 64ull, 2, 64, 64, 2, 1, 2) : get_map(&p.mapB, w, 192ull, 64ull, 0, 64, 64, 0, 1, 2);
+    constexpr unsigned long long K = G::KB * 64ull;
+    int rc = SPLIT ? get_map(&p.mapB, w, K, 64ull, 2, 64, 64, 2, 1, 2) : get_map(&p.mapB, w, K, 64ull, 0, 64, 64, 0, 1, 2);
     if (rc) return rc;
     p.plane = out * 64;
     p.x = x; p.bias = bias; p.y = static_cast<__half*>(y);
     static bool attr[64] = {false};
     const int dev = current_device();
     if (!attr[dev]) {
-        RF_CUDA(cudaFuncSetAttribute(stem7_kernel<SPLIT>, cudaFuncAttributeMaxDynamicSharedMemorySize, ST_SMEM));
+        RF_CUDA(cudaFuncSetAttribute(stem_kernel<KS, S, SPLIT>, cudaFuncAttributeMaxDynamicSharedMemorySize, G::SMEM));
         attr[dev] = true;
     }
-    const int grid = units < num_sms() ? units : num_sms();
-    stem7_kernel<SPLIT><<<grid, ST_THREADS, ST_SMEM, as_stream(stream)>>>(p);
+    const int resident = G::CTAS * num_sms();
+    stem_kernel<KS, S, SPLIT><<<units < resident ? units : resident, ST_THREADS, G::SMEM, as_stream(stream)>>>(p);
     RF_LAUNCHED();
     return 0;
 }
@@ -936,8 +972,13 @@
     return conv_impl(set, p, w_split, as_stream(stream), K_SPLIT, false, &dual);
 }
 
-int rf_stem7(ActFormat f, const float* x, int nimg, const int* hw_host, const void* w, const float* bias, int pool, void* y, void* stream) {
-    return f == ACT_SPLIT ? stem_impl<true>(x, nimg, hw_host, w, bias, y, pool, stream) : stem_impl<false>(x, nimg, hw_host, w, bias, y, pool, stream);
+int rf_stem(ActFormat f, const float* x, int nimg, const int* hw_host, int k, int stride, const void* w, const float* bias, int pool, void* y,
+            void* stream) {
+    const bool split = f == ACT_SPLIT;
+    if (k == 7 && stride == 2)
+        return split ? stem_impl<7, 2, true>(x, nimg, hw_host, w, bias, y, pool, stream) : stem_impl<7, 2, false>(x, nimg, hw_host, w, bias, y, pool, stream);
+    RF_REQUIRE(k == 3 && stride == 1 && !pool, "rf_stem: the 7x7 / stride 2 stem (optionally pooled) or the 3x3 / stride 1 stem");
+    return split ? stem_impl<3, 1, true>(x, nimg, hw_host, w, bias, y, 0, stream) : stem_impl<3, 1, false>(x, nimg, hw_host, w, bias, y, 0, stream);
 }
 
 size_t rf_corr_tc_workspace(int NA, int NB, int C) { return 2ull * ((size_t)NA + NB) * C * sizeof(float) + 1024; }
diff --git a/ransac-flow_b200/csrc/runner.cu b/ransac-flow_b200/csrc/runner.cu
--- a/ransac-flow_b200/csrc/runner.cu
+++ b/ransac-flow_b200/csrc/runner.cu
@@ -6,7 +6,8 @@
 int rf_blur(ActFormat f, const void* x, int nimg, const int* hw_host, int C, int stride, void* y, void* stream);
 int rf_poolblur(ActFormat f, const void* x, int nimg, const int* hw_host, int C, void* y, void* stream);
 int rf_im2col(ActFormat f, const float* x, int nimg, const int* hw_host, int C, int k, int stride, int pad, int Kpad, void* y, void* stream);
-int rf_stem7(ActFormat f, const float* x, int nimg, const int* hw_host, const void* w, const float* bias, int pool, void* y, void* stream);
+int rf_stem(ActFormat f, const float* x, int nimg, const int* hw_host, int k, int stride, const void* w, const float* bias, int pool, void* y,
+            void* stream);
 int rf_stem3(const float* x, int nimg, const int* hw_host, const float* w, const float* bias, void* y, void* stream);
 int rf_conv2d_nhwc_dil(const float* x, int nimg, const int* hw_host, int Cin, const float* w, const float* w_tc, const float* bias,
                        const float* residual, int Cout, int R, int S, int stride, int pad, int dil, int relu, int engine, float* y, void* stream);
@@ -58,14 +59,15 @@
             break;
         case RF_OP_STEM7: {
             RF_REQUIRE(f == ACT_F16 || f == ACT_SPLIT, "rf_run_layers: RF_OP_STEM7 needs engine 2 or 4");
-            RF_REQUIRE(l.src == L[0].src && l.Cin == 3 && l.Cout == 64 && k == 7 && stride == 2 && pad == 3 && l.relu,
-                       "rf_run_layers: RF_OP_STEM7 is the ResNet-50 stem on the fp32 input slot");
+            RF_REQUIRE(l.src == L[0].src && l.Cin == 3 && l.Cout == 64 && ((k == 7 && stride == 2 && pad == 3) || (k == 3 && stride == 1 && pad == 1)) && l.relu,
+                       "rf_run_layers: RF_OP_STEM7 is the ResNet-50 stem (7x7 / 2 / pad 3) or the FeatureExtractor stem (3x3 / 1 / pad 1) on the fp32 input slot");
             const bool pool = (l.flags & RF_LAYER_STEM_POOL) != 0;
+            RF_REQUIRE(!pool || k == 7, "rf_run_layers: RF_LAYER_STEM_POOL pools the 7x7 stem");
             const rf_layer_t* mp = pool && li + 1 < n ? &L[li + 1] : nullptr;
             RF_REQUIRE(!pool || (mp != nullptr && mp->op == RF_OP_MAXPOOL && mp->src == l.dst && mp->Cin == 64 && mp->k == 3 && mp->stride == 2 &&
                                  mp->pad == 1 && mp->dst >= 0 && mp->dst < RF_MAX_SLOTS && mp->dst != l.src),
                        "rf_run_layers: RF_LAYER_STEM_POOL needs the next layer to be a 3x3 / stride 2 / pad 1 max-pool of the stem's output");
-            rc = rf_stem7(f, x, nimg, shw, l.w_f16, l.bias, pool, pool ? slots[mp->dst] : y, stream);
+            rc = rf_stem(f, x, nimg, shw, k, stride, l.w_f16, l.bias, pool, pool ? slots[mp->dst] : y, stream);
             if (rc) return rc;
             if (pool) {
                 for (int i = 0; i < nimg; ++i)
diff --git a/ransac-flow_b200/csrc/wgmma.cuh b/ransac-flow_b200/csrc/wgmma.cuh
--- a/ransac-flow_b200/csrc/wgmma.cuh
+++ b/ransac-flow_b200/csrc/wgmma.cuh
@@ -35,6 +35,14 @@
         : "l"(a), "l"(b));
 }
 
+__device__ __forceinline__ void wgmma_f16_n64_rs(float (&d)[32], const uint32_t (&a)[4], uint64_t b) {
+    asm volatile(
+        "{\n\t.reg .pred p;\n\tsetp.ne.b32 p, 1, 0;\n\t"
+        "wgmma.mma_async.sync.aligned.m64n64k16.f32.f16.f16 {%0, %1, %2, %3, %4, %5, %6, %7, %8, %9, %10, %11, %12, %13, %14, %15, %16, %17, %18, %19, %20, %21, %22, %23, %24, %25, %26, %27, %28, %29, %30, %31}, {%32, %33, %34, %35}, %36, p, 1, 1, 0;\n\t}"
+        : "+f"(d[0]), "+f"(d[1]), "+f"(d[2]), "+f"(d[3]), "+f"(d[4]), "+f"(d[5]), "+f"(d[6]), "+f"(d[7]), "+f"(d[8]), "+f"(d[9]), "+f"(d[10]), "+f"(d[11]), "+f"(d[12]), "+f"(d[13]), "+f"(d[14]), "+f"(d[15]), "+f"(d[16]), "+f"(d[17]), "+f"(d[18]), "+f"(d[19]), "+f"(d[20]), "+f"(d[21]), "+f"(d[22]), "+f"(d[23]), "+f"(d[24]), "+f"(d[25]), "+f"(d[26]), "+f"(d[27]), "+f"(d[28]), "+f"(d[29]), "+f"(d[30]), "+f"(d[31])
+        : "r"(a[0]), "r"(a[1]), "r"(a[2]), "r"(a[3]), "l"(b));
+}
+
 template <bool TF32, int N>
 __device__ __forceinline__ void wgmma(float (&d)[N / 2], uint64_t a, uint64_t b) {
     if constexpr (TF32) { if constexpr (N == 64) wgmma_tf32_n64(d, a, b); else wgmma_tf32_n128(d, a, b); }
diff --git a/ransac-flow_b200/model.py b/ransac-flow_b200/model.py
--- a/ransac-flow_b200/model.py
+++ b/ransac-flow_b200/model.py
@@ -174,7 +174,10 @@
 
     def _fold_build(self, f16=False):
         P = LayerProgram(3)
-        x = P.stem(0, self.conv1.weight, self.bn1, 1, 1, 64 if f16 else 32)
+        if f16:
+            x = P.stem7_fused(0, self.conv1.weight, self.bn1)
+        else:
+            x = P.stem(0, self.conv1.weight, self.bn1, 1, 1)
         x = P.poolblur(x)
         for layer in (self.layer1, self.layer2, self.layer3):
             for b in layer:
diff --git a/ransac-flow_b200/program.py b/ransac-flow_b200/program.py
--- a/ransac-flow_b200/program.py
+++ b/ransac-flow_b200/program.py
@@ -85,12 +85,14 @@
     def stem7_fused(self, src, weight, bn):
         from .model import FoldedConv
         cout, cin, k, _ = weight.shape
-        assert (cout, cin, k) == (64, 3, 7) and self.chan[src] == 3
+        assert (cout, cin) == (64, 3) and k in (7, 3) and self.chan[src] == 3
+        stride, pad = (2, 3) if k == 7 else (1, 1)
+        kpad = (k * k * cin + 63) // 64 * 64
         dev = self.device or weight.device
         w = weight.detach().float().cpu().permute(0, 2, 3, 1).reshape(cout, k * k * cin)
-        w = torch.nn.functional.pad(w, (0, 192 - k * k * cin)).reshape(cout, 192, 1, 1)
+        w = torch.nn.functional.pad(w, (0, kpad - k * k * cin)).reshape(cout, kpad, 1, 1)
         fc = FoldedConv(w, bn, 1, pad=0, device=dev)
-        self.ops.append((RF_OP_STEM7, src, -1, 3, 64, 7, 2, 3, 1, fc))
+        self.ops.append((RF_OP_STEM7, src, -1, 3, 64, k, stride, pad, 1, fc))
         self._keep.append(fc)
         self.chan.append(64)
         self.f16_only = True
@@ -140,7 +142,7 @@
         stem_pool = set()
         for i, o in enumerate(self.ops[:-1]):
             q = self.ops[i + 1]
-            if (f16 or split) and o[0] == RF_OP_STEM7 and q[0] == RF_OP_MAXPOOL and q[1] == i + 1 and tuple(q[5:8]) == (3, 2, 1) \
+            if (f16 or split) and o[0] == RF_OP_STEM7 and o[5] == 7 and q[0] == RF_OP_MAXPOOL and q[1] == i + 1 and tuple(q[5:8]) == (3, 2, 1) \
                     and last_use[i + 1] == i + 1:
                 stem_pool.add(i)
                 elems[i + 1] = 0
```

Measured after the change: 146.9, median of 6. +3.7%, better.
